# WeaponizedSchizophrenia/physically-based-renderer

Hardware: AMD Instinct MI355X
Metric: Mpaths/s + HBM GB/s (% of peak), 1920x1080x1024 spp glTF scene (higher is better)
Workload: dtype f32

## Files before the change

physically-based-renderer_amd/csrc/pt_kernels.hip:

```cpp
#include "pt_device.h"
#include "ptc_internal.h"

#ifndef TRACE_BLOCK
#define TRACE_BLOCK 256
#endif
#ifndef TRACE_MIN_WAVES
#define TRACE_MIN_WAVES 8
#endif
#define TRACE_WAVES (TRACE_BLOCK / 64)
#ifndef TRACE_CHUNK
#define TRACE_CHUNK 512u
#endif
#ifndef TRACE_CHUNK_SHORT
#define TRACE_CHUNK_SHORT 64u
#endif
#ifndef TRACE_REFILL_IDLE
#define TRACE_REFILL_IDLE 1
#endif
#ifndef TRACE_RING
#define TRACE_RING 64
#endif
#define RING_FIELDS 5
#ifndef TRACE_NODE_MIN
#define TRACE_NODE_MIN 40
#endif
#ifndef TRACE_NODE_MIN_ANY
#define TRACE_NODE_MIN_ANY TRACE_NODE_MIN
#endif
#ifndef SHADE_BLOCK
#define SHADE_BLOCK 256
#endif
#ifndef SHADE_MIN_WAVES
#define SHADE_MIN_WAVES 4
#endif
#define SHADE_WAVES (SHADE_BLOCK / 64)
#define SHADE_LDS_LIGHTS 64
#define SHADE_LDS_MATS 64
#define SHADE_LDS_ENV_ROWS 2048
#define HIT_CLASS_SHIFT 28

PT_DEV uint32_t wave_fetch(uint32_t* ctr, uint32_t amount, uint32_t lane) {
  uint32_t base = 0;
  if (lane == 0) base = atomicAdd(ctr, amount);
  return (uint32_t)__builtin_amdgcn_readfirstlane((int)base);
}
PT_DEV unsigned long long wave_sum(unsigned long long v) {
  for (int o = 32; o > 0; o >>= 1) v += __shfl_xor(v, o);
  return v;
}

#define SCAN_BLOCK 1024
PT_DEV uint32_t block_sum_1024(uint32_t v, uint32_t* s_w , uint32_t& excl) {
  const uint32_t lane = lane_id(), wave = threadIdx.x >> 6;
  uint32_t inc = v;
#pragma unroll
  for (int o = 1; o < 64; o <<= 1) { const uint32_t t = __shfl_up(inc, o); if ((int)lane >= o) inc += t; }
  __syncthreads();
  if (lane == 63) s_w[wave] = inc;
  __syncthreads();
  uint32_t before = 0, total = 0;
#pragma unroll
  for (uint32_t w = 0; w < SCAN_BLOCK / 64; ++w) { const uint32_t t = s_w[w]; if (w < wave) before += t; total += t; }
  excl = before + inc - v;
  return total;
}
PT_DEV void scan_chunks(const uint32_t* seg, uint32_t n_seg, uint32_t* pre, uint32_t* hdr, uint32_t trace_waves, uint32_t* s_w) {
  const uint32_t per = (n_seg + SCAN_BLOCK - 1u) / SCAN_BLOCK;
  const uint32_t s0 = threadIdx.x * per, s1 = s0 + per < n_seg ? s0 + per : n_seg;
  uint32_t mine = 0, dummy;
  for (uint32_t sg = s0; sg < s1; ++sg) mine += seg[sg];
  const uint32_t total = block_sum_1024(mine, s_w, dummy);
  const uint32_t per_wave = (total + trace_waves - 1u) / trace_waves;
  const uint32_t chunk = per_wave >= TRACE_CHUNK ? TRACE_CHUNK : TRACE_CHUNK_SHORT;
  uint32_t chunks = 0;
  for (uint32_t sg = s0; sg < s1; ++sg) chunks += (seg[sg] + chunk - 1u) / chunk;
  uint32_t run;
  const uint32_t all = block_sum_1024(chunks, s_w, run);
  for (uint32_t sg = s0; sg < s1; ++sg) { pre[sg] = run; run += (seg[sg] + chunk - 1u) / chunk; }
  if (threadIdx.x == 0) { pre[n_seg] = all; hdr[0] = total; hdr[1] = chunk; hdr[2] = all; }
}
__global__ __launch_bounds__(SCAN_BLOCK) void k_set_counts(DevQueues q, uint32_t n_rays, uint32_t n_shadow, uint32_t trace_waves) {
  __shared__ uint32_t s_w[SCAN_BLOCK / 64];
  for (uint32_t sg = threadIdx.x; sg < q.n_seg; sg += SCAN_BLOCK) {
    const uint64_t lo = (uint64_t)sg * q.seg_len;
    q.seg_ray[0][sg] = lo >= n_rays ? 0u : (n_rays - lo > q.seg_len ? q.seg_len : (uint32_t)(n_rays - lo));
    q.seg_ray[1][sg] = 0u;
    q.seg_sh[sg] = lo >= n_shadow ? 0u : (n_shadow - lo > q.seg_len ? q.seg_len : (uint32_t)(n_shadow - lo));
  }
  __syncthreads();
  scan_chunks(q.seg_ray[0], q.n_seg, q.pre_ray, &q.cnt[CNT_RAY_TOTAL], trace_waves, s_w);
  scan_chunks(q.seg_sh, q.n_seg, q.pre_sh, &q.cnt[CNT_SH_TOTAL], trace_waves, s_w);
  if (threadIdx.x == 0) { q.cnt[CNT_WORK_TRACE] = 0; q.cnt[CNT_WORK_SHADOW] = 0; }
}
__global__ __launch_bounds__(SCAN_BLOCK) void k_scan(DevQueues q, int qi_next, uint32_t trace_waves) {
  __shared__ uint32_t s_w[SCAN_BLOCK / 64];
  scan_chunks(q.seg_ray[qi_next], q.n_seg, q.pre_ray, &q.cnt[CNT_RAY_TOTAL], trace_waves, s_w);
  scan_chunks(q.seg_sh, q.n_seg, q.pre_sh, &q.cnt[CNT_SH_TOTAL], trace_waves, s_w);
  if (threadIdx.x == 0) { q.cnt[CNT_WORK_TRACE] = 0; q.cnt[CNT_WORK_SHADOW] = 0; }
}

template <bool RASTER>
__global__ __launch_bounds__(256) void k_raygen(DevCamera cam, DevFrame fr, DevQueues q, uint32_t first_sample, uint32_t n_paths) {
  const uint32_t p = blockIdx.x * 256u + threadIdx.x;
  if (p >= n_paths) return;
  const uint32_t j = p % fr.n_owned, sl = p / fr.n_owned;
  const uint32_t pixel = fr.owned[j];
  const uint32_t px = pixel % (uint32_t)fr.w, py = pixel / (uint32_t)fr.w;
  const uint32_t sample = first_sample + sl;
  const uint32_t key = path_key(fr.seed_hash, pixel, sample);
  float jx = 0.5f, jy = 0.5f;
  if (!RASTER) { jx = rng_f(key, 0, 0); jy = rng_f(key, 0, 1); }
  const float fx = ((float)px + jx) / (float)fr.w, fy = ((float)py + jy) / (float)fr.h;
  const float dvx = (2.0f * fx - 1.0f) * cam.sx, dvy = (2.0f * fy - 1.0f) * cam.sy;
  const v3 cs = V3(cam.s[0], cam.s[1], cam.s[2]), cu = V3(cam.u[0], cam.u[1], cam.u[2]), cf = V3(cam.f[0], cam.f[1], cam.f[2]);
  const v3 d = normalize3(vfma(cs, dvx, vfma(cu, dvy, cf)));
  float bz = 1.0f, bw = 1.0f;
  if (RASTER) {
    const float len = pt_sqrt(pt_fma(dvy, dvy, pt_fma(dvx, dvx, 1.0f)));
    const float dnear = (2.0f * PT_ZFAR * PT_ZNEAR) / (PT_ZFAR + PT_ZNEAR);
    bz = dnear * len; bw = PT_ZFAR * len;
  }
  const RayQ& r = q.ray[0];
  r.A[p] = make_float4(cam.pos[0], cam.pos[1], cam.pos[2], d.x);
  r.B[p] = make_float4(d.y, d.z, bz, bw);
  r.C[p] = make_float4(1.0f, 0.0f, __uint_as_float(p), __uint_as_float(key));
  q.lpath[p] = make_float4(0.0f, 0.0f, 0.0f, 0.0f);
}

struct WStack {
  typedef unsigned int ux2 __attribute__((ext_vector_type(2)));
  typedef __attribute__((address_space(3))) ux2 lds_u2;
  typedef __attribute__((address_space(1))) ux2 glb_u2;
  lds_u2* lds; glb_u2* ovf; int sp; int L;
  PT_DEV void init(uint2* lds_base, uint2* ovf_wave, int l) { lds = (lds_u2*)lds_base; ovf = (glb_u2*)ovf_wave; sp = 0; L = l; }
  PT_DEV void reset() { sp = 0; }
  PT_DEV void push(uint32_t base, uint32_t mask) {
    const ux2 e = {base, mask};
    if (sp < L) lds[sp * 64] = e; else ovf[(sp - L) * 64 + (int)lane_id()] = e;
    ++sp;
  }
  PT_DEV uint2 pop() {
    --sp;
    ux2 e;
    if (sp < L) e = lds[sp * 64]; else e = ovf[(sp - L) * 64 + (int)lane_id()];
    return make_uint2(e.x, e.y);
  }
  PT_DEV bool empty() const { return sp == 0; }
};

typedef float float2v __attribute__((ext_vector_type(2)));
PT_DEV float hw_max(float a, float b) { return __builtin_fmaxf(a, b); }
PT_DEV float hw_min(float a, float b) { return __builtin_fminf(a, b); }
PT_DEV float ubyte_f(uint32_t w, int i) { return (float)((w >> (8 * i)) & 255u); }

#define CUR_DONE ((int)0x80000000)
#define CUR_FINISHED (CUR_DONE + 1)
#define CUR_LEAF (CUR_DONE + 2)

PT_DEV uint32_t ray_octant(const ray_t& r) { return (r.inv.x >= 0.0f ? 1u : 0u) | (r.inv.y >= 0.0f ? 2u : 0u) | (r.inv.z >= 0.0f ? 4u : 0u); }

#define ORDER_TABLE_BYTES 2048
PT_DEV void build_order_table(uint8_t* tab) {
  for (uint32_t i = threadIdx.x; i < ORDER_TABLE_BYTES; i += TRACE_BLOCK) {
    const uint32_t oct = i >> 8, hits = i & 255u;
    uint32_t best = 0, bk = 0;
    for (uint32_t sl = 0; sl < 8u; ++sl)
      if ((hits >> sl) & 1u) { const uint32_t k = (sl ^ oct) + 1u; if (k > bk) { bk = k; best = sl; } }
    tab[i] = (uint8_t)best;
  }
}

PT_DEV uint32_t node_visit(const DevScene& sc, uint32_t node_addr, int cur, const ray_t& r, uint32_t oct, float tmin, float tlimit,
                           uint32_t& block, uint32_t& masks) {
  typedef float fx4 __attribute__((ext_vector_type(4)));
  typedef __attribute__((address_space(3))) const fx4 lds_f4;
  typedef __attribute__((address_space(1))) const fx4 glb_f4;
  fx4 f0, f1, f2, f3;
  if ((uint32_t)cur < sc.n_lds_units) {
    lds_f4* p = (lds_f4*)(uintptr_t)node_addr;
    f0 = p[0]; f1 = p[1]; f2 = p[2]; f3 = p[3];
  } else {
    glb_f4* p = (glb_f4*)sc.recs + (uint32_t)cur;
    f0 = p[0]; f1 = p[1]; f2 = p[2]; f3 = p[3];
  }
  const uint32_t w0 = __float_as_uint(f0.x), w1 = __float_as_uint(f0.y), w2 = __float_as_uint(f0.z);
  const float ox = pt_fma((float)(w0 & 0xffffu), sc.grid_step[0], sc.grid_lo[0]), oy = pt_fma((float)(w0 >> 16), sc.grid_step[1], sc.grid_lo[1]),
              oz = pt_fma((float)(w1 & 0xffffu), sc.grid_step[2], sc.grid_lo[2]);
  const float ax = __uint_as_float(((w1 >> 16) & 255u) << 23) * r.inv.x, ay = __uint_as_float((w1 >> 24) << 23) * r.inv.y,
              az = __uint_as_float((w2 & 255u) << 23) * r.inv.z;
  const float bx = pt_fma(ox, r.inv.x, -(r.o.x * r.inv.x)), by = pt_fma(oy, r.inv.y, -(r.o.y * r.inv.y)), bz = pt_fma(oz, r.inv.z, -(r.o.z * r.inv.z));
  const bool px = (oct & 1u) != 0u, py = (oct & 2u) != 0u, pz = (oct & 4u) != 0u;
  const uint32_t lx[2] = {__float_as_uint(f1.x), __float_as_uint(f1.y)}, ly[2] = {__float_as_uint(f1.z), __float_as_uint(f1.w)},
                 lz[2] = {__float_as_uint(f2.x), __float_as_uint(f2.y)}, hx[2] = {__float_as_uint(f2.z), __float_as_uint(f2.w)},
                 hy[2] = {__float_as_uint(f3.x), __float_as_uint(f3.y)}, hz[2] = {__float_as_uint(f3.z), __float_as_uint(f3.w)};
  uint32_t hits = 0;
#pragma unroll
  for (int h = 1; h >= 0; --h) {
    const uint32_t nqx = px ? lx[h] : hx[h], fqx = px ? hx[h] : lx[h];
    const uint32_t nqy = py ? ly[h] : hy[h], fqy = py ? hy[h] : ly[h];
    const uint32_t nqz = pz ? lz[h] : hz[h], fqz = pz ? hz[h] : lz[h];
#pragma unroll
    for (int i = 3; i >= 0; --i) {
      const float tn = hw_max(hw_max(hw_max(pt_fma(ubyte_f(nqx, i), ax, bx), pt_fma(ubyte_f(nqy, i), ay, by)), pt_fma(ubyte_f(nqz, i), az, bz)), tmin);
      const float tf = hw_min(hw_min(hw_min(pt_fma(ubyte_f(fqx, i), ax, bx), pt_fma(ubyte_f(fqy, i), ay, by)), pt_fma(ubyte_f(fqz, i), az, bz)), tlimit);
#ifndef PT_NO_ADDC
// ... 33 lines not shown
  const uint32_t second = tmask >> 24;
  const uint32_t k = tbase + 3u * ((uint32_t)__builtin_popcount((tmask >> 8) & 255u & below) + (uint32_t)__builtin_popcount((tmask >> 16) & 255u & below) + second);
  const bool more = second == 0u && ((tmask >> (16u + sl)) & 1u) != 0u;
  tmask = more ? (tmask | (1u << 24)) : ((tmask & 0x00ffffffu) & ~(1u << sl));
  return k;
}

PT_DEV uint32_t pending_triangles(uint32_t tmask) {
  const uint32_t lh = tmask & 255u;
  return (uint32_t)__builtin_popcount(lh) + (uint32_t)__builtin_popcount((tmask >> 16) & lh) - (tmask >> 24);
}
#ifndef LEAF_EXTRA
#define LEAF_EXTRA 1
#endif
struct LeafDeal { uint32_t off, take, ntask, rank_free; bool helper; };
PT_DEV LeafDeal leaf_deal(uint32_t extra, bool leaf, uint64_t m_leaf) {
  LeafDeal d;
  uint32_t off = 0, total = 0;
#pragma unroll
  for (int b = 0; (1 << b) <= LEAF_EXTRA; ++b) {
    const uint64_t m = __ballot(((extra >> b) & 1u) != 0u);
    off += mbcnt64(m) << b; total += (uint32_t)__popcll(m) << b;
  }
  const uint64_t m_free = ~m_leaf;
  const uint32_t n_free = (uint32_t)__popcll(m_free);
  d.rank_free = mbcnt64(m_free);
  d.ntask = total < n_free ? total : n_free;
  d.helper = !leaf && d.rank_free < d.ntask;
  d.off = off;
  d.take = off >= d.ntask ? 0u : (d.ntask - off < extra ? d.ntask - off : extra);
  return d;
}

struct Reservoir {
  uint32_t next, end, n_chunks, chunk, my_static; bool exhausted, static_left;
  PT_DEV void init(const uint32_t* hdr, uint32_t wave_in_grid) {
    chunk = hdr[1]; n_chunks = hdr[2];
    my_static = wave_in_grid; static_left = wave_in_grid < n_chunks;
    next = end = 0; exhausted = false;
  }
  static PT_DEV bool block_has_no_work(const uint32_t* hdr) { return hdr[2] <= blockIdx.x * TRACE_WAVES; }
  PT_DEV void open_chunk(const DevQueues& q, const uint32_t* pre, const uint32_t* seg, uint32_t c, uint32_t lane) {
    uint32_t lo = 0, span = q.n_seg;
    while (span > 1u) {
      const uint32_t step = (span + 63u) >> 6, idx = lo + lane * step;
      const uint32_t v = lane * step < span ? pre[idx] : 0xffffffffu;
      const uint32_t k = (uint32_t)__popcll(__ballot(v <= c)) - 1u;
      lo += k * step;
      span = span - k * step < step ? span - k * step : step;
    }
    const uint32_t first = pre[lo], cnt = seg[lo];
    const uint32_t j = c - (uint32_t)__builtin_amdgcn_readfirstlane((int)first), live = (uint32_t)__builtin_amdgcn_readfirstlane((int)cnt);
    lo = (uint32_t)__builtin_amdgcn_readfirstlane((int)lo);
    next = lo * q.seg_len + j * chunk;
    end = lo * q.seg_len + ((j + 1u) * chunk < live ? (j + 1u) * chunk : live);
  }
  PT_DEV uint32_t take(const DevQueues& q, const uint32_t* pre, const uint32_t* seg, uint32_t* ctr, uint32_t lane, uint32_t want, uint32_t& first) {
    if (next >= end && !exhausted) {
      if (chunk < TRACE_CHUNK) {
        if (my_static < n_chunks) { open_chunk(q, pre, seg, my_static, lane); my_static += gridDim.x * TRACE_WAVES; }
        else exhausted = true;
      } else if (static_left) { static_left = false; open_chunk(q, pre, seg, my_static, lane); }
      else {
        const uint32_t waves = gridDim.x * TRACE_WAVES;
        if (n_chunks <= waves) exhausted = true;
        else {
          const uint64_t c = (uint64_t)waves + wave_fetch(ctr, 1u, lane);
          if (c >= n_chunks) exhausted = true; else open_chunk(q, pre, seg, (uint32_t)c, lane);
        }
      }
    }
    const uint32_t avail = end - next;
    const uint32_t n = avail < want ? avail : want;
    first = next; next += n;
    return n;
  }
};

struct RayRing {
  typedef __attribute__((address_space(3))) uint32_t lds_u32;
  lds_u32* f;
  uint32_t n;
  PT_DEV void init(uint32_t* base) { f = (lds_u32*)base; n = 0; }
  PT_DEV void stage(Reservoir& res, const DevQueues& q, const uint32_t* pre, const uint32_t* seg, uint32_t* ctr, const float4* QA, const float4* QB, uint32_t lane) {
    uint32_t first;
    const uint32_t k = res.take(q, pre, seg, ctr, lane, TRACE_RING, first);
    if (lane < k) {
      const uint32_t ri = first + lane;
      const float4 A = QA[ri], B = QB[ri];
      const ray_t r = make_ray(V3(A.x, A.y, A.z), V3(A.w, B.x, B.y));
      f[lane] = ri;
      f[TRACE_RING + lane] = __float_as_uint(r.inv.x); f[2 * TRACE_RING + lane] = __float_as_uint(r.inv.y); f[3 * TRACE_RING + lane] = __float_as_uint(r.inv.z);
      f[4 * TRACE_RING + lane] = (r.inv.x >= 0.0f ? 1u : 0u) | (r.inv.y >= 0.0f ? 2u : 0u) | (r.inv.z >= 0.0f ? 4u : 0u);
    }
    n = (uint32_t)__builtin_amdgcn_readfirstlane((int)k);
    __builtin_amdgcn_fence(__ATOMIC_RELEASE, "wavefront");
    __builtin_amdgcn_wave_barrier();
    __builtin_amdgcn_fence(__ATOMIC_ACQUIRE, "wavefront");
  }
  PT_DEV bool pop(bool idle, uint32_t& ri, v3& inv, uint32_t& oct) {
    const uint64_t m = __ballot(idle);
    const uint32_t rank = mbcnt64(m), need = (uint32_t)__popcll(m);
    const bool got = idle && rank < n;
    if (got) {
      const uint32_t i = n - 1u - rank;
      ri = f[i];
      inv = V3(__uint_as_float(f[TRACE_RING + i]), __uint_as_float(f[2 * TRACE_RING + i]), __uint_as_float(f[3 * TRACE_RING + i]));
      oct = f[4 * TRACE_RING + i];
    }
    n -= need < n ? need : n;
    return got;
  }
};

#ifdef PT_DIAG
#define DIAG_ITER(var) do { const uint64_t m_ = __ballot(true); if ((int)lane == __ffsll((unsigned long long)m_) - 1) ++(var); } while (0)
#else
#define DIAG_ITER(var) do { } while (0)
#endif

struct TraceLds { uint32_t top_addr; uint2* stack; uint8_t* order_tab; uint32_t* ring; };
PT_DEV TraceLds trace_lds(float4* lds_raw, const DevScene& sc, int stack_lds, bool closest) {
  TraceLds t;
  t.top_addr = (uint32_t)(uintptr_t)(__attribute__((address_space(3))) void*)lds_raw;
  t.stack = reinterpret_cast<uint2*>(lds_raw + sc.n_lds_units);
  t.order_tab = reinterpret_cast<uint8_t*>(t.stack + (size_t)TRACE_WAVES * (size_t)stack_lds * 64u);
  t.ring = reinterpret_cast<uint32_t*>(t.order_tab + (closest ? ORDER_TABLE_BYTES : 0));
  return t;
}
PT_DEV void load_triangle(const DevScene& sc, uint32_t top_addr, uint32_t k, float4& a, float4& b, float4& c) {
  typedef float fx4 __attribute__((ext_vector_type(4)));
  typedef __attribute__((address_space(3))) const fx4 lds_f4;
  typedef __attribute__((address_space(1))) const fx4 glb_f4;
  fx4 x, y, z;
  if (k + 3u <= sc.n_lds_units) { lds_f4* p = (lds_f4*)(uintptr_t)(top_addr + 16u * k); x = p[0]; y = p[1]; z = p[2]; }
  else { glb_f4* p = (glb_f4*)sc.recs + k; x = p[0]; y = p[1]; z = p[2]; }
  a = make_float4(x.x, x.y, x.z, x.w); b = make_float4(y.x, y.y, y.z, y.w); c = make_float4(z.x, z.y, z.z, z.w);
}

template <bool CULL>
__global__ __launch_bounds__(TRACE_BLOCK, TRACE_MIN_WAVES) void k_trace_closest(DevScene sc, DevQueues q, int qi, int stack_lds) {
  extern __shared__ float4 lds_raw[];
  __shared__ uint8_t s_pair[2][TRACE_WAVES][64];
  const uint32_t lane = lane_id();
  const uint32_t wave = threadIdx.x >> 6;
  if (Reservoir::block_has_no_work(&q.cnt[CNT_RAY_TOTAL])) return;
  const TraceLds L = trace_lds(lds_raw, sc, stack_lds, true);
  uint8_t* order_tab = L.order_tab;
  for (uint32_t i = threadIdx.x; i < sc.n_lds_units; i += TRACE_BLOCK) lds_raw[i] = sc.recs[i];
  build_order_table(order_tab);
  __syncthreads();
  const RayQ rq = q.ray[qi];
  unsigned long long nv = 0, nr = 0, nh = 0;
  uint32_t nt = 0;
  uint32_t d_node = 0, d_tri = 0, d_round = 0, d_leftpass = 0, d_left = 0;
  (void)d_node; (void)d_tri; (void)d_round; (void)d_leftpass; (void)d_left;
#ifdef PT_STAMP
  unsigned long long t_refill = 0, t_node = 0, t_leaf = 0, t_fin = 0, t_mark = __builtin_amdgcn_s_memtime();
#define STAMP(acc) do { __builtin_amdgcn_sched_barrier(0); const unsigned long long t_ = __builtin_amdgcn_s_memtime(); acc += t_ - t_mark; t_mark = t_; __builtin_amdgcn_sched_barrier(0); } while (0)
#else
#define STAMP(acc) do { } while (0)
#endif
  Reservoir res; res.init(&q.cnt[CNT_RAY_TOTAL], (uint32_t)__builtin_amdgcn_readfirstlane((int)(blockIdx.x * TRACE_WAVES + wave)));
  const uint32_t* seg_cnt = q.seg_ray[qi];
  WStack st;
  st.init(L.stack + (size_t)wave * (size_t)stack_lds * 64u + lane,
          sc.stack_ovf + ((size_t)__builtin_amdgcn_readfirstlane((int)(blockIdx.x * TRACE_WAVES + wave)) * sc.ovf_depth) * 64u, stack_lds);
  int cur = CUR_DONE;
  uint32_t ri = 0, oct = 0, gbase = 0, gmask = 0, tbase = 0, tmask = 0;
  ray_t r = make_ray(V3(0, 0, 0), V3(0, 0, 1));
  float tmin = 0.0f, best_t = PT_T_INF, best_u = 0.0f, best_v = 0.0f;
  int best_prim = 0x7fffffff, best_cls = 0;
  bool found = false;
  RayRing ring; ring.init(L.ring + (size_t)wave * RING_FIELDS * TRACE_RING);
  for (;;) {
    {
      bool idle = cur == CUR_DONE;
      uint64_t mi = __ballot(idle);
      if ((uint32_t)__popcll(mi) >= TRACE_REFILL_IDLE || !__ballot(cur != CUR_DONE)) {
        while (mi) {
          if (ring.n == 0u) {
            if (res.exhausted) break;
            ring.stage(res, q, q.pre_ray, seg_cnt, &q.cnt[CNT_WORK_TRACE], rq.A, rq.B, lane);
            if (ring.n == 0u) break;
          }
          v3 inv = V3(0, 0, 0); uint32_t oc = 0;
          const bool got = ring.pop(idle, ri, inv, oc);
          nr += (unsigned long long)__popcll(__ballot(got));
          if (got) {
            const float4 A = rq.A[ri], Bq = rq.B[ri];
            r.o = V3(A.x, A.y, A.z); r.d = V3(A.w, Bq.x, Bq.y); r.inv = inv;
            oct = oc;
            tmin = CULL ? Bq.z : 0.0f;
            best_t = CULL ? Bq.w : PT_T_INF; best_u = 0.0f; best_v = 0.0f; best_prim = 0x7fffffff; best_cls = 0; found = false;
            st.reset();
            gmask = 0; tmask = 0;
            cur = 0;
          }
          idle = cur == CUR_DONE; mi = __ballot(idle);
        }
      }
    }
    STAMP(t_refill);
    if (!__ballot(cur != CUR_DONE)) break;
    DIAG_ITER(d_round);
    {
      for (;;) {
        const uint64_t mn = __ballot(cur >= 0);
        if (!mn) break;
        if (__popcll(mn) < TRACE_NODE_MIN && __ballot(cur == CUR_LEAF)) break;
        nv += (unsigned long long)__popcll(mn);
        if (cur >= 0) {
          DIAG_ITER(d_node);
          uint32_t nb, masks;
          const uint32_t node_addr = L.top_addr + 16u * (uint32_t)cur;
          const uint32_t hits = node_visit(sc, node_addr, cur, r, oct, tmin, best_t, nb, masks);
          const uint32_t imask = masks & 255u, lhits = hits & (masks >> 8);
          enter_group(gbase, gmask, st, nb, hits & imask, imask);
          tbase = nb + 4u * (uint32_t)__builtin_popcount(imask);
          tmask = lhits | (masks & 0x00ffff00u);
          cur = lhits ? CUR_LEAF : advance<true>(gbase, gmask, st, order_tab, oct);
        }
      }
      STAMP(t_node);
#if LEAF_EXTRA == 0
      {
        const bool leaf = cur == CUR_LEAF;
        if (__ballot(leaf)) {
          DIAG_ITER(d_tri);
          if (leaf) {
            const uint32_t k = next_triangle(tbase, tmask);
            float4 a, b, c;
            load_triangle(sc, L.top_addr, k, a, b, c);
            float t, u, v;
            const bool hit = tri_test<CULL>(r, V3(a.x, a.y, a.z), V3(b.x, b.y, b.z), V3(c.x, c.y, c.z), t, u, v);
            const int pid = __float_as_int(a.w);
            ++nt;
            if (hit && t > tmin && (t < best_t || (t == best_t && pid < best_prim))) {
              best_t = t; best_u = u; best_v = v; best_prim = pid; best_cls = __float_as_int(b.w); found = true;
            }
            if ((tmask & 255u) == 0u) cur = advance<true>(gbase, gmask, st, order_tab, oct);
          }
        }
      }
#elif LEAF_EXTRA > 1
      {
        const bool leaf = cur == CUR_LEAF;
        const uint64_t m_leaf = __ballot(leaf);
        if (m_leaf) {
          DIAG_ITER(d_tri);
          uint32_t k1 = 0, pend = 0;
          if (leaf) { k1 = next_triangle(tbase, tmask); pend = pending_triangles(tmask); }
          const LeafDeal dl = leaf_deal(pend < LEAF_EXTRA ? pend : LEAF_EXTRA, leaf, m_leaf);
          typedef __attribute__((address_space(3))) volatile uint8_t lds_u8;
          lds_u8* tab_task = (lds_u8*)s_pair[0][wave];
          lds_u8* tab_helper = (lds_u8*)s_pair[1][wave];
          uint32_t kx[LEAF_EXTRA];
#pragma unroll
          for (uint32_t j = 0; j < LEAF_EXTRA; ++j) {
            kx[j] = 0;
            if (j < dl.take) { kx[j] = next_triangle(tbase, tmask); tab_task[dl.off + j] = (uint8_t)(lane | (j << 6)); }
          }
          if (dl.helper) tab_helper[dl.rank_free] = (uint8_t)lane;
          __builtin_amdgcn_fence(__ATOMIC_RELEASE, "wavefront");
          __builtin_amdgcn_wave_barrier();
          __builtin_amdgcn_fence(__ATOMIC_ACQUIRE, "wavefront");
          const uint32_t task = dl.helper ? (uint32_t)tab_task[dl.rank_free] : lane;
          const int src = (int)(task & 63u);
          ray_t rr;
          rr.o = V3(__shfl(r.o.x, src), __shfl(r.o.y, src), __shfl(r.o.z, src));
          rr.d = V3(__shfl(r.d.x, src), __shfl(r.d.y, src), __shfl(r.d.z, src));
          uint32_t k = k1;
#pragma unroll
          for (uint32_t j = 0; j < LEAF_EXTRA; ++j) {
            const uint32_t kj = (uint32_t)__shfl((int)kx[j], src);
            if (dl.helper && (task >> 6) == j) k = kj;
          }
          bool hit = false; float t = 0.0f, u = 0.0f, v = 0.0f; int pid = 0, cls = 0;
          if (leaf || dl.helper) {
            float4 a, b, c;
            load_triangle(sc, L.top_addr, k, a, b, c);
            hit = tri_test<CULL>(rr, V3(a.x, a.y, a.z), V3(b.x, b.y, b.z), V3(c.x, c.y, c.z), t, u, v);
            pid = __float_as_int(a.w); cls = __float_as_int(b.w);
          }
          if (leaf) {
            ++nt;
            if (hit && t > tmin && (t < best_t || (t == best_t && pid < best_prim))) {
              best_t = t; best_u = u; best_v = v; best_prim = pid; best_cls = cls; found = true;
            }
          }
          const float tt = hit ? t : -INFINITY;
          const int pw = pid | (cls << HIT_CLASS_SHIFT);
          float bt = 0.0f; int bp = 0, bl = (int)lane; bool have = false;
#pragma unroll
          for (uint32_t j = 0; j < LEAF_EXTRA; ++j) {
            const int hl = j < dl.take ? (int)tab_helper[dl.off + j] : (int)lane;
            const float tj = __shfl(tt, hl);
            const int pj = __shfl(pw, hl);
            if (j < dl.take) {
              ++nt;
              const int prim_j = pj & ((1 << HIT_CLASS_SHIFT) - 1);
              if (tj > tmin && (!have || tj < bt || (tj == bt && prim_j < (bp & ((1 << HIT_CLASS_SHIFT) - 1))))) { bt = tj; bp = pj; bl = hl; have = true; }
            }
          }
          const float ub = __shfl(u, bl), vb = __shfl(v, bl);
          if (have) {
            const int prim_b = bp & ((1 << HIT_CLASS_SHIFT) - 1);
            if (bt < best_t || (bt == best_t && prim_b < best_prim)) {
              best_t = bt; best_u = ub; best_v = vb; best_prim = prim_b; best_cls = (int)((uint32_t)bp >> HIT_CLASS_SHIFT); found = true;
            }
          }
          if (leaf && (tmask & 255u) == 0u) cur = advance<true>(gbase, gmask, st, order_tab, oct);
#ifdef PT_DIAG
          {
            const uint32_t left = (cur == CUR_LEAF) ? pending_triangles(tmask) : 0u;
            const uint64_t m_left = __ballot(left != 0u);
            if (m_left) { if ((int)lane == __ffsll((unsigned long long)m_left) - 1) ++d_leftpass; d_left += left; }
          }
#endif
        }
      }
#else
      {
        const bool leaf = cur == CUR_LEAF;
        const uint64_t m_leaf = __ballot(leaf);
        if (m_leaf) {
          DIAG_ITER(d_tri);
          uint32_t k1 = 0, k2 = 0;
          bool more = false;
          if (leaf) { k1 = next_triangle(tbase, tmask); more = (tmask & 255u) != 0u; }
          const uint64_t m_more = __ballot(more), m_free = ~m_leaf;
          const uint32_t n_more = (uint32_t)__popcll(m_more), n_free = (uint32_t)__popcll(m_free);
          const uint32_t rank_more = mbcnt64(m_more), rank_free = mbcnt64(m_free);
          const bool paired = more && rank_more < n_free, helper = !leaf && rank_free < n_more;
          typedef __attribute__((address_space(3))) volatile uint8_t lds_u8;
          lds_u8* tab_owner = (lds_u8*)s_pair[0][wave];
          lds_u8* tab_helper = (lds_u8*)s_pair[1][wave];
          if (paired) { k2 = next_triangle(tbase, tmask); tab_owner[rank_more] = (uint8_t)lane; }
          if (helper) tab_helper[rank_free] = (uint8_t)lane;
          __builtin_amdgcn_fence(__ATOMIC_RELEASE, "wavefront");
          __builtin_amdgcn_wave_barrier();
          __builtin_amdgcn_fence(__ATOMIC_ACQUIRE, "wavefront");
          const int src = helper ? (int)tab_owner[rank_free] : (int)lane;
          ray_t rr;
          rr.o = V3(__shfl(r.o.x, src), __shfl(r.o.y, src), __shfl(r.o.z, src));
          rr.d = V3(__shfl(r.d.x, src), __shfl(r.d.y, src), __shfl(r.d.z, src));
          const uint32_t k2_src = (uint32_t)__shfl((int)k2, src);
          const uint32_t k = helper ? k2_src : k1;
          bool hit = false; float t = 0.0f, u = 0.0f, v = 0.0f; int pid = 0, cls = 0;
          if (leaf || helper) {
            float4 a, b, c;
            load_triangle(sc, L.top_addr, k, a, b, c);
            hit = tri_test<CULL>(rr, V3(a.x, a.y, a.z), V3(b.x, b.y, b.z), V3(c.x, c.y, c.z), t, u, v);
            pid = __float_as_int(a.w); cls = __float_as_int(b.w);
          }
          if (leaf) {
            ++nt;
            if (hit && t > tmin && (t < best_t || (t == best_t && pid < best_prim))) {
              best_t = t; best_u = u; best_v = v; best_prim = pid; best_cls = cls; found = true;
            }
          }
          const int hsrc = paired ? (int)tab_helper[rank_more] : (int)lane;
          const int h2 = __shfl(hit ? 1 : 0, hsrc);
          const float t2 = __shfl(t, hsrc), u2 = __shfl(u, hsrc), v2 = __shfl(v, hsrc);
          const int pid2 = __shfl(pid, hsrc), cls2 = __shfl(cls, hsrc);
          if (paired) {
            ++nt;
            if (h2 && t2 > tmin && (t2 < best_t || (t2 == best_t && pid2 < best_prim))) {
              best_t = t2; best_u = u2; best_v = v2; best_prim = pid2; best_cls = cls2; found = true;
            }
          }
          if (leaf && (tmask & 255u) == 0u) cur = advance<true>(gbase, gmask, st, order_tab, oct);
#ifdef PT_DIAG
          {
            const uint32_t left = (cur == CUR_LEAF) ? (uint32_t)__builtin_popcount(tmask & 255u) + (uint32_t)__builtin_popcount((tmask >> 16) & tmask & 255u) - (tmask >> 24) : 0u;
            const uint64_t m_left = __ballot(left != 0u);
            if (m_left) { if ((int)lane == __ffsll((unsigned long long)m_left) - 1) ++d_leftpass; d_left += left; }
          }
#endif
        }
      }
#endif
      STAMP(t_leaf);
      nh += (unsigned long long)__popcll(__ballot(cur == CUR_FINISHED && found));
      if (cur == CUR_FINISHED) {
        q.hit[ri] = make_float4(found ? best_t : -1.0f, __int_as_float(found ? (best_prim | (best_cls << HIT_CLASS_SHIFT)) : -1), best_u, best_v);
        cur = CUR_DONE;
      }
      STAMP(t_fin);
    }
  }
  {
    __shared__ unsigned long long s_stat[TRACE_WAVES][4];
    const unsigned long long c_tris = wave_sum(nt);
    if (lane == 0) { s_stat[wave][0] = nv; s_stat[wave][1] = c_tris; s_stat[wave][2] = nr; s_stat[wave][3] = nh; }
    __syncthreads();
    if (threadIdx.x < 4u) {
      unsigned long long v = 0;
      for (int w = 0; w < TRACE_WAVES; ++w) v += s_stat[w][threadIdx.x];
      const int at = threadIdx.x == 0u ? ST_NODES_C : threadIdx.x == 1u ? ST_TRIS_C : threadIdx.x == 2u ? ST_SEGMENTS : ST_HITS;
      if (v) atomicAdd(&q.stats[at * ST_STRIDE], v);
    }
  }
#ifdef PT_STAMP
  if (lane == 0) { atomicAdd(&q.stats[ST_DIAG_NODE_ITERS * ST_STRIDE], t_node); atomicAdd(&q.stats[ST_DIAG_TRI_ITERS * ST_STRIDE], t_leaf); atomicAdd(&q.stats[ST_DIAG_LEAF_VISITS * ST_STRIDE], t_fin); atomicAdd(&q.stats[ST_DIAG_ROUNDS * ST_STRIDE], t_refill); }
#endif
#ifdef PT_DIAG
  {
    unsigned long long a0 = wave_sum(d_node), a1 = wave_sum(d_tri), a3 = wave_sum(d_round), a4 = wave_sum(d_leftpass), a5 = wave_sum(d_left);
    if (lane == 0) { atomicAdd(&q.stats[ST_DIAG_NODE_ITERS * ST_STRIDE], a0); atomicAdd(&q.stats[ST_DIAG_TRI_ITERS * ST_STRIDE], a1); atomicAdd(&q.stats[ST_DIAG_ROUNDS * ST_STRIDE], a3);
                     atomicAdd(&q.stats[ST_DIAG_LEAF_VISITS * ST_STRIDE], a4); atomicAdd(&q.stats[ST_DIAG_REFILLED * ST_STRIDE], a5); }
  }
#endif
}

template <bool DEBUG_OUT>
__global__ __launch_bounds__(TRACE_BLOCK, TRACE_MIN_WAVES) void k_trace_any(DevScene sc, DevQueues q, int stack_lds, uint8_t* debug_out) {
  extern __shared__ float4 lds_raw[];
  __shared__ uint8_t s_pair[2][TRACE_WAVES][64];
  const uint32_t lane = lane_id();
  const uint32_t wave = threadIdx.x >> 6;
  if (Reservoir::block_has_no_work(&q.cnt[CNT_SH_TOTAL])) return;
  const TraceLds L = trace_lds(lds_raw, sc, stack_lds, false);
  for (uint32_t i = threadIdx.x; i < sc.n_lds_units; i += TRACE_BLOCK) lds_raw[i] = sc.recs[i];
  __syncthreads();
  unsigned long long nv = 0, nr = 0;
  uint32_t nt = 0;
  Reservoir res; res.init(&q.cnt[CNT_SH_TOTAL], (uint32_t)__builtin_amdgcn_readfirstlane((int)(blockIdx.x * TRACE_WAVES + wave)));
  WStack st;
  st.init(L.stack + (size_t)wave * (size_t)stack_lds * 64u + lane,
          sc.stack_ovf + ((size_t)__builtin_amdgcn_readfirstlane((int)(blockIdx.x * TRACE_WAVES + wave)) * sc.ovf_depth) * 64u, stack_lds);
  int cur = CUR_DONE;
  uint32_t ri = 0, path = 0, oct = 0, gbase = 0, gmask = 0, tbase = 0, tmask = 0;
  ray_t r = make_ray(V3(0, 0, 0), V3(0, 0, 1));
  float tmax = 0.0f;
  bool occluded = false;
  RayRing ring; ring.init(L.ring + (size_t)wave * RING_FIELDS * TRACE_RING);
  for (;;) {
    {
      bool idle = cur == CUR_DONE;
      uint64_t mi = __ballot(idle);
      if ((uint32_t)__popcll(mi) >= TRACE_REFILL_IDLE || !__ballot(cur != CUR_DONE)) {
        while (mi) {
          if (ring.n == 0u) {
            if (res.exhausted) break;
            ring.stage(res, q, q.pre_sh, q.seg_sh, &q.cnt[CNT_WORK_SHADOW], q.shadow.A, q.shadow.B, lane);
            if (ring.n == 0u) break;
          }
          v3 inv = V3(0, 0, 0); uint32_t oc = 0;
          const bool got = ring.pop(idle, ri, inv, oc);
          nr += (unsigned long long)__popcll(__ballot(got));
          if (got) {
            const float4 A = q.shadow.A[ri], Bq = q.shadow.B[ri];
            r.o = V3(A.x, A.y, A.z); r.d = V3(A.w, Bq.x, Bq.y); r.inv = inv;
            oct = oc;
            tmax = Bq.z; path = __float_as_uint(Bq.w);
            occluded = false;
            st.reset();
            gmask = 0; tmask = 0;
            cur = 0;
          }
          idle = cur == CUR_DONE; mi = __ballot(idle);
        }
      }
    }
    if (!__ballot(cur != CUR_DONE)) break;
    {
      for (;;) {
        const uint64_t mn = __ballot(cur >= 0);
        if (!mn) break;
        if (__popcll(mn) < TRACE_NODE_MIN_ANY && __ballot(cur == CUR_LEAF)) break;
        nv += (unsigned long long)__popcll(mn);
        if (cur >= 0) {
          uint32_t nb, masks;
          const uint32_t node_addr = L.top_addr + 16u * (uint32_t)cur;
          const uint32_t hits = node_visit(sc, node_addr, cur, r, oct, 0.0f, tmax, nb, masks);
          const uint32_t imask = masks & 255u, lhits = hits & (masks >> 8);
          enter_group(gbase, gmask, st, nb, hits & imask, imask);
          tbase = nb + 4u * (uint32_t)__builtin_popcount(imask);
          tmask = lhits | (masks & 0x00ffff00u);
          cur = lhits ? CUR_LEAF : advance<false>(gbase, gmask, st, nullptr, 0u);
        }
      }
#if LEAF_EXTRA == 0
      {
        const bool leaf = cur == CUR_LEAF;
        if (__ballot(leaf)) {
          if (leaf) {
            const uint32_t k = next_triangle(tbase, tmask);
            float4 a, b, c;
            load_triangle(sc, L.top_addr, k, a, b, c);
            float t, u, v;
            const bool hit = tri_test<false>(r, V3(a.x, a.y, a.z), V3(b.x, b.y, b.z), V3(c.x, c.y, c.z), t, u, v) && t > 0.0f && t < tmax;
            ++nt;
            if (hit) { occluded = true; cur = CUR_FINISHED; }
            else if ((tmask & 255u) == 0u) cur = advance<false>(gbase, gmask, st, nullptr, 0u);
          }
        }
      }
#elif LEAF_EXTRA > 1
      {
        const bool leaf = cur == CUR_LEAF;
        const uint64_t m_leaf = __ballot(leaf);
        if (m_leaf) {
          uint32_t k1 = 0, pend = 0;
          if (leaf) { k1 = next_triangle(tbase, tmask); pend = pending_triangles(tmask); }
          const LeafDeal dl = leaf_deal(pend < LEAF_EXTRA ? pend : LEAF_EXTRA, leaf, m_leaf);
          typedef __attribute__((address_space(3))) volatile uint8_t lds_u8;
          lds_u8* tab_task = (lds_u8*)s_pair[0][wave];
          lds_u8* tab_helper = (lds_u8*)s_pair[1][wave];
          uint32_t kx[LEAF_EXTRA];
#pragma unroll
          for (uint32_t j = 0; j < LEAF_EXTRA; ++j) {
            kx[j] = 0;
            if (j < dl.take) { kx[j] = next_triangle(tbase, tmask); tab_task[dl.off + j] = (uint8_t)(lane | (j << 6)); }
          }
          if (dl.helper) tab_helper[dl.rank_free] = (uint8_t)lane;
          __builtin_amdgcn_fence(__ATOMIC_RELEASE, "wavefront");
          __builtin_amdgcn_wave_barrier();
          __builtin_amdgcn_fence(__ATOMIC_ACQUIRE, "wavefront");
          const uint32_t task = dl.helper ? (uint32_t)tab_task[dl.rank_free] : lane;
          const int src = (int)(task & 63u);
          ray_t rr;
          rr.o = V3(__shfl(r.o.x, src), __shfl(r.o.y, src), __shfl(r.o.z, src));
          rr.d = V3(__shfl(r.d.x, src), __shfl(r.d.y, src), __shfl(r.d.z, src));
          const float tmax_src = __shfl(tmax, src);
          uint32_t k = k1;
#pragma unroll
          for (uint32_t j = 0; j < LEAF_EXTRA; ++j) {
// ... 183 lines not shown
  if (y0 < 0) y0 += si.z;
  if (x1 > si.y - 1) x1 -= si.y;
  if (y1 > si.z - 1) y1 -= si.z;
  const uint4 t00 = ldu4(sc.set_texels, set_texel_at(si, x0, y0)), t10 = ldu4(sc.set_texels, set_texel_at(si, x1, y0)),
              t01 = ldu4(sc.set_texels, set_texel_at(si, x0, y1)), t11 = ldu4(sc.set_texels, set_texel_at(si, x1, y1));
  auto bil = [&](uint32_t p00, uint32_t p10, uint32_t p01, uint32_t p11) {
    const float4 c00 = unorm8x4(p00), c10 = unorm8x4(p10), c01 = unorm8x4(p01), c11 = unorm8x4(p11);
    const float ax = pt_fma(tx, c10.x - c00.x, c00.x), ay = pt_fma(tx, c10.y - c00.y, c00.y), az = pt_fma(tx, c10.z - c00.z, c00.z), aw = pt_fma(tx, c10.w - c00.w, c00.w);
    const float bx = pt_fma(tx, c11.x - c01.x, c01.x), by = pt_fma(tx, c11.y - c01.y, c01.y), bz = pt_fma(tx, c11.z - c01.z, c01.z), bw = pt_fma(tx, c11.w - c01.w, c01.w);
    return make_float4(pt_fma(ty, bx - ax, ax), pt_fma(ty, by - ay, ay), pt_fma(ty, bz - az, az), pt_fma(ty, bw - aw, aw));
  };
  c = bil(t00.x, t10.x, t01.x, t11.x); n = bil(t00.y, t10.y, t01.y, t11.y); m = bil(t00.z, t10.z, t01.z, t11.z);
}

template <class S> PT_DEV void apply_textures(const S& sc, float4 t0, float4 t1, float4 t2, float4 t3, float4 t4, float4 t5, float hu, float hv, float hw, float4 M2, int set, v3 ni, float base[4],
                           float& metallic, float& roughness, v3& ns) {
  const int tex_color = __float_as_int(M2.y), tex_normal = __float_as_int(M2.z), tex_mr = __float_as_int(M2.w);
  const float tu = pt_fma(t1.x, hv, pt_fma(t0.z, hu, t0.x * hw)), tv = pt_fma(t1.y, hv, pt_fma(t0.w, hu, t0.y * hw));
  float4 cc = make_float4(1, 1, 1, 1), cn = make_float4(0.5f, 0.5f, 1.0f, 1.0f), cm = make_float4(1, 1, 1, 1);
  const int4 si = ldi4(sc.set_info, (size_t)(set < 0 ? 0 : set));
  if (set >= 0 && si.x >= 0) set_fetch(sc, si, tu, tv, cc, cn, cm);
  else {
    if (tex_color >= 0) cc = tex_fetch(sc, tex_color, tu, tv);
    if (tex_mr >= 0) cm = tex_fetch(sc, tex_mr, tu, tv);
    if (tex_normal >= 0) cn = tex_fetch(sc, tex_normal, tu, tv);
  }
  if (tex_color >= 0) { base[0] = base[0] * cc.x; base[1] = base[1] * cc.y; base[2] = base[2] * cc.z; base[3] = base[3] * cc.w; }
  if (tex_mr >= 0) { roughness = roughness * cm.y; metallic = metallic * cm.z; }
  if (tex_normal >= 0) {
    const float nx = 2.0f * cn.x - 1.0f, ny = 2.0f * cn.y - 1.0f, nz = 2.0f * cn.z - 1.0f;
    const v3 ti = V3(pt_fma(t3.x, hv, pt_fma(t2.y, hu, t1.z * hw)), pt_fma(t3.y, hv, pt_fma(t2.z, hu, t1.w * hw)), pt_fma(t3.z, hv, pt_fma(t2.w, hu, t2.x * hw)));
    const v3 bi = V3(pt_fma(t5.y, hv, pt_fma(t4.z, hu, t3.w * hw)), pt_fma(t5.z, hv, pt_fma(t4.w, hu, t4.x * hw)), pt_fma(t5.w, hv, pt_fma(t5.x, hu, t4.y * hw)));
    ns = normalize3(vfma(ti, nx, vfma(bi, ny, ni * nz)));
  }
}

template <class S> PT_DEV void env_lookup(const S& sc, v3 d, v3& Le, float& pdf) {
  const float u = pt_atan2(d.z, d.x) * (0.5f * PT_INV_PI) + 0.5f;
  const float dy = fmin2(fmax2(d.y, -1.0f), 1.0f);
  const float st = pt_sqrt(fmax2(0.0f, 1.0f - dy * dy));
  const float vv = pt_atan2(st, dy) * PT_INV_PI;
  int x = (int)(u * (float)sc.env_w), y = (int)(vv * (float)sc.env_h);
  if (x > sc.env_w - 1) x = sc.env_w - 1;
  if (x < 0) x = 0;
  if (y > sc.env_h - 1) y = sc.env_h - 1;
  if (y < 0) y = 0;
  const float4 t = ld4(sc.env, (size_t)y * (size_t)sc.env_w + (size_t)x);
  Le = V3(t.x, t.y, t.z);
  pdf = sc.env_ok ? (t.w * (float)sc.env_w * (float)sc.env_h) / (2.0f * PT_PI * PT_PI * fmax2(st, 1e-6f)) : 0.0f;
}
template <class P> PT_DEV uint32_t cdf_search(const P& cdf, uint32_t n, float r) {
  uint32_t lo = 0, hi = n - 1u;
  while (lo < hi) { const uint32_t mid = (lo + hi) >> 1; if (cdf[mid] > r) hi = mid; else lo = mid + 1u; }
  return lo;
}
template <class P, class G> PT_DEV uint32_t cdf_search_guided(const P& cdf, const G& guide, float r) {
  const uint32_t b = (uint32_t)(r * (float)PTC_ENV_GUIDE);
  uint32_t lo = guide[b], hi = guide[b + 1u];
  while (lo < hi) { const uint32_t mid = (lo + hi) >> 1; if (cdf[mid] > r) hi = mid; else lo = mid + 1u; }
  return lo;
}
template <class S, class P, class G> PT_DEV v3 env_sample(const S& sc, const P& marg, const G& marg_guide, float r1, float r2) {
  const uint32_t y = cdf_search_guided(marg, marg_guide, r1);
  const float m0 = y ? marg[y - 1u] : 0.0f, m1 = marg[y];
  float xi_v = m1 > m0 ? (r1 - m0) / (m1 - m0) : 0.5f;
  const auto cc = sc.env_cond + (size_t)y * (size_t)sc.env_w;
  const uint32_t x = cdf_search_guided(cc, sc.env_cond_guide + (size_t)y * (PTC_ENV_GUIDE + 1u), r2);
  const float c0 = x ? cc[x - 1u] : 0.0f, c1 = cc[x];
  float xi_u = c1 > c0 ? (r2 - c0) / (c1 - c0) : 0.5f;
  xi_u = fmin2(fmax2(xi_u, 0.0f), 0.999999f); xi_v = fmin2(fmax2(xi_v, 0.0f), 0.999999f);
  const float u = ((float)x + xi_u) / (float)sc.env_w, vv = ((float)y + xi_v) / (float)sc.env_h;
  float s2, c2, st, ct;
  sincos2pi(u, s2, c2);
  sincos2pi(0.5f * vv, st, ct);
  return V3(st * -c2, ct, st * -s2);
}

#define SHADE_RING 128
PT_DEV void wave_lds_sync() {
  __builtin_amdgcn_fence(__ATOMIC_RELEASE, "wavefront");
  __builtin_amdgcn_wave_barrier();
  __builtin_amdgcn_fence(__ATOMIC_ACQUIRE, "wavefront");
}
template <bool SORT, bool TABLES_LDS>
__global__ __launch_bounds__(SHADE_BLOCK, SHADE_MIN_WAVES) void k_shade(const DevScene* __restrict__ scp, DevFrame fr, DevQueues q, int qi, uint32_t b) {
  __shared__ float4 s_light[SHADE_LDS_LIGHTS * 5];
  __shared__ float s_cdf[SHADE_LDS_LIGHTS];
  __shared__ float4 s_mat[SHADE_LDS_MATS * 4];
  __shared__ uint32_t s_ring[SORT ? SHADE_WAVES : 1][PTC_MATERIAL_CLASSES][SORT ? SHADE_RING : 1];
  __shared__ float s_marg[SHADE_LDS_ENV_ROWS];
  __shared__ uint16_t s_marg_guide[PTC_ENV_GUIDE + 2];
  const DevScene& dsc = *scp;
  const GScene sc = global_view(dsc);
  const uint32_t lane = lane_id();
  const uint32_t wave = threadIdx.x >> 6;
  const bool lds_lights = TABLES_LDS || sc.n_lights <= SHADE_LDS_LIGHTS, lds_mats = TABLES_LDS || sc.n_mats <= SHADE_LDS_MATS;
  if (lds_lights) {
    for (uint32_t i = threadIdx.x; i < sc.n_lights * 5u; i += SHADE_BLOCK) s_light[i] = ld4((AS_GLOBAL const fx4*)dsc.lights, i);
    for (uint32_t i = threadIdx.x; i < sc.n_lights; i += SHADE_BLOCK) s_cdf[i] = ((AS_GLOBAL const float*)dsc.cdf)[i];
  }
  if (lds_mats)
    for (uint32_t i = threadIdx.x; i < sc.n_mats * 4u; i += SHADE_BLOCK) s_mat[i] = ld4((AS_GLOBAL const fx4*)dsc.mats, i);
  const bool lds_marg = sc.env_ok != 0 && (TABLES_LDS || sc.env_h <= SHADE_LDS_ENV_ROWS);
  if (lds_marg) {
    for (uint32_t i = threadIdx.x; i < (uint32_t)sc.env_h; i += SHADE_BLOCK) s_marg[i] = ((AS_GLOBAL const float*)dsc.env_marg)[i];
    for (uint32_t i = threadIdx.x; i <= PTC_ENV_GUIDE; i += SHADE_BLOCK) s_marg_guide[i] = ((AS_GLOBAL const uint16_t*)dsc.env_marg_guide)[i];
  }
  __syncthreads();
  const Dual<float, TABLES_LDS> env_marg = {(AS_LDS const float*)s_marg, (AS_GLOBAL const float*)dsc.env_marg, lds_marg};
  const Dual<uint16_t, TABLES_LDS> env_marg_guide = {(AS_LDS const uint16_t*)s_marg_guide, (AS_GLOBAL const uint16_t*)dsc.env_marg_guide, lds_marg};
  const uint32_t seg = blockIdx.x * SHADE_WAVES + wave;
  if (seg >= q.n_seg) return;
  const Dual<fx4, TABLES_LDS> lights = {(AS_LDS const fx4*)s_light, (AS_GLOBAL const fx4*)dsc.lights, lds_lights};
  const Dual<float, TABLES_LDS> cdf = {(AS_LDS const float*)s_cdf, (AS_GLOBAL const float*)dsc.cdf, lds_lights};
  const Dual<fx4, TABLES_LDS> mats = {(AS_LDS const fx4*)s_mat, (AS_GLOBAL const fx4*)dsc.mats, lds_mats};
  const bool has_env = sc.env_w > 0, env_nee = has_env && sc.env_ok != 0;
  const float p_env = env_nee ? (sc.n_lights > 0u ? 0.5f : 1.0f) : 0.0f, p_area = 1.0f - p_env;
  const RayQ rin = q.ray[qi], rout = q.ray[qi ^ 1];
  const uint32_t base = seg * q.seg_len;
  const uint32_t n = (uint32_t)__builtin_amdgcn_readfirstlane((int)q.seg_ray[qi][seg]);
  typedef __attribute__((address_space(3))) volatile uint32_t lds_u32;
  lds_u32* ring = (lds_u32*)&s_ring[SORT ? wave : 0][0][0];
#ifdef PT_STAMP_SHADE
  unsigned long long t_front = 0, t_load = 0, t_math = 0, t_back = 0, t_mark = __builtin_amdgcn_s_memtime();
#define SSTAMP(acc) do { __builtin_amdgcn_sched_barrier(0); const unsigned long long t_ = __builtin_amdgcn_s_memtime(); acc += t_ - t_mark; t_mark = t_; __builtin_amdgcn_sched_barrier(0); } while (0)
#define SSTAMP_LOADS(acc) do { asm volatile("s_waitcnt vmcnt(0)" ::: "memory"); SSTAMP(acc); } while (0)
#else
#define SSTAMP(acc) do { } while (0)
#define SSTAMP_LOADS(acc) do { } while (0)
#endif
  uint32_t out_a = 0, out_s = 0;
  uint32_t fillv = 0;
  uint32_t ready = 0, nonempty = 0;
  uint32_t i0 = 0;
  int w_pref = SORT && lane < n ? __float_as_int(q.hit[base + lane].y) : -1;
  for (;;) {
    bool valid; uint32_t item = 0u;
    if (!SORT) {
      if (i0 >= n) break;
      valid = i0 + lane < n; item = i0 + lane;
      i0 += 64u;
    } else {
    if (!ready) {
      if (i0 < n) {
        const uint32_t i = i0 + lane;
        int cls = -1;
        if (i < n) cls = w_pref >= 0 ? ((w_pref >> HIT_CLASS_SHIFT) & (PTC_MATERIAL_CLASSES - 1)) : (has_env ? PTC_MATERIAL_CLASSES - 1 : -1);
#ifdef SHADE_TWO_RING
        if (cls >= 0) cls = (cls >= 2 && cls != PTC_MATERIAL_CLASSES - 1) ? 1 : 0;
#endif
        i0 += 64u;
        w_pref = i0 + lane < n ? __float_as_int(q.hit[base + i0 + lane].y) : -1;
        uint64_t rem = __ballot(cls >= 0);
        while (rem) {
          const int c = __builtin_amdgcn_readlane(cls, __ffsll((unsigned long long)rem) - 1);
          const uint64_t m = __ballot(cls == c);
          uint32_t f = (uint32_t)__builtin_amdgcn_readlane((int)fillv, c);
          if (cls == c) ring[(uint32_t)c * SHADE_RING + f + mbcnt64(m)] = i;
          f += (uint32_t)__popcll(m);
          if (lane == (uint32_t)c) fillv = f;
          nonempty |= 1u << c;
          if (f >= 64u) ready |= 1u << c;
          rem &= ~m;
        }
        SSTAMP(t_front);
        continue;
      }
      if (!nonempty) break;
    }
    wave_lds_sync();
    if (ready) {
      const uint32_t c = (uint32_t)__builtin_ctz(ready);
      const uint32_t f = (uint32_t)__builtin_amdgcn_readlane((int)fillv, (int)c);
      const uint32_t rest = f - 64u;
      valid = true;
      item = ring[c * SHADE_RING + rest + lane];
      if (lane == c) fillv = rest;
      ready &= ~(1u << c);
      if (!rest) nonempty &= ~(1u << c);
    } else {
      uint32_t off = 0, left = nonempty;
      valid = false;
      while (left && off < 64u) {
        const uint32_t c = (uint32_t)__builtin_ctz(left);
        const uint32_t f = (uint32_t)__builtin_amdgcn_readlane((int)fillv, (int)c);
        const uint32_t take = f < 64u - off ? f : 64u - off;
        if (lane >= off && lane < off + take) { item = ring[c * SHADE_RING + f - take + (lane - off)]; valid = true; }
        if (lane == c) fillv = f - take;
        if (f == take) nonempty &= ~(1u << c);
        left &= ~(1u << c);
        off += take;
      }
    }
    }
    const uint32_t slot = base + item;
    SSTAMP(t_front);

    bool alive = false, has_shadow = false;
    float4 oA, oB, oC, sA, sB, sC;
    oA = oB = oC = sA = sB = sC = make_float4(0, 0, 0, 0);
    if (valid) {
      const float4 A = rin.A[slot], Bq = rin.B[slot], Cq = rin.C[slot], H = q.hit[slot];
      const v3 d = V3(A.w, Bq.x, Bq.y);
      v3 T = V3(Bq.z, Bq.w, Cq.x);
      const float prev_pdf = Cq.y;
      const uint32_t path = __float_as_uint(Cq.z), key = __float_as_uint(Cq.w);
      const float ht = H.x, hu = H.z, hv = H.w;
      if (__float_as_int(H.y) < 0) {
        if (SORT || has_env) {
        v3 Le; float pe; env_lookup(sc, d, Le, pe);
        float wgt = 1.0f;
        if (b > 0u) { const float pl = pe * p_env; const float pb2 = prev_pdf * prev_pdf; wgt = pb2 / pt_fma(pl, pl, pb2); }
        float4 L = q.lpath[path];
        L.x = pt_fma(T.x * Le.x, wgt, L.x); L.y = pt_fma(T.y * Le.y, wgt, L.y); L.z = pt_fma(T.z * Le.z, wgt, L.z);
        q.lpath[path] = L;
        }
      } else {
      const uint32_t prim = (uint32_t)__float_as_int(H.y) & ((1u << HIT_CLASS_SHIFT) - 1u);
      const size_t rec = (size_t)prim * sc.shade_stride;
      const float4 r0 = ld4(sc.shade, rec), r1 = ld4(sc.shade, rec + 1), r2 = ld4(sc.shade, rec + 2), r3 = ld4(sc.shade, rec + 3), r4 = ld4(sc.shade, rec + 4);
      const bool tex_cls = ((uint32_t)__float_as_int(H.y) >> HIT_CLASS_SHIFT) >= 2u;
      float4 x0, x1, x2, x3, x4, x5;
      x0 = x1 = x2 = x3 = x4 = x5 = make_float4(0, 0, 0, 0);
      if (tex_cls) { x0 = ld4(sc.shade, rec + 5); x1 = ld4(sc.shade, rec + 6); x2 = ld4(sc.shade, rec + 7); x3 = ld4(sc.shade, rec + 8); x4 = ld4(sc.shade, rec + 9); x5 = ld4(sc.shade, rec + 10); }
      const uint32_t rb = b + 1u;
      bool use_env = false;
      if ((int)b < fr.max_bounces && env_nee) use_env = sc.n_lights == 0u || rng_f(key, rb, 7) < p_env;
      v3 wi_env = V3(0, 0, 0);
#ifdef SHADE_ENV_ALWAYS
      if ((int)b < fr.max_bounces && env_nee) wi_env = env_sample(sc, env_marg, env_marg_guide, rng_f(key, rb, 1), rng_f(key, rb, 2));
#else
      if (use_env) wi_env = env_sample(sc, env_marg, env_marg_guide, rng_f(key, rb, 1), rng_f(key, rb, 2));
#endif
      SSTAMP_LOADS(t_load);
      const v3 Pa = V3(r0.x, r0.y, r0.z), Pb = V3(r1.x, r1.y, r1.z), Pc = V3(r2.x, r2.y, r2.z);
      const v3 Na = V3(r2.w, r3.x, r3.y), Nb = V3(r3.z, r3.w, r4.x), Nc = V3(r4.y, r4.z, r4.w);
      const float hw = 1.0f - hu - hv;
      const v3 P = V3(pt_fma(Pc.x, hv, pt_fma(Pb.x, hu, Pa.x * hw)), pt_fma(Pc.y, hv, pt_fma(Pb.y, hu, Pa.y * hw)), pt_fma(Pc.z, hv, pt_fma(Pb.z, hu, Pa.z * hw)));
      v3 ng = normalize3(cross3(Pb - Pa, Pc - Pa));
      const v3 ni = V3(pt_fma(Nc.x, hv, pt_fma(Nb.x, hu, Na.x * hw)), pt_fma(Nc.y, hv, pt_fma(Nb.y, hu, Na.y * hw)), pt_fma(Nc.z, hv, pt_fma(Nb.z, hu, Na.z * hw)));
      v3 ns = normalize3(ni);
      const int mat = __float_as_int(r0.w);
      const float4 M0 = ld4(mats, (size_t)(mat * 4 + 0)), M1 = ld4(mats, (size_t)(mat * 4 + 1)), M2 = ld4(mats, (size_t)(mat * 4 + 2));
      float base_c[4] = {M0.x, M0.y, M0.z, M2.x};
      float metallic = M0.w, roughness = M1.w;
      const bool lambert = metallic == 0.0f && roughness >= 1.0f && __float_as_int(M2.w) < 0;
      if (__float_as_int(M2.y) >= 0 || __float_as_int(M2.z) >= 0 || __float_as_int(M2.w) >= 0)
        apply_textures(sc, x0, x1, x2, x3, x4, x5, hu, hv, hw, M2, __float_as_int(ld4(mats, (size_t)(mat * 4 + 3)).x), ni, base_c, metallic, roughness, ns);
      const v3 wo = -d;
      const bool front = dot3(ng, wo) > 0.0f;
      if (dot3(ns, ng) < 0.0f) ns = -ns;
      if (!front) { ng = -ng; ns = -ns; }
      if (!(dot3(ns, wo) > 0.0f)) ns = ng;
      const int li = __float_as_int(r1.w);
      if (li >= 0 && front) {
        const float4 l0 = ld4(lights, (size_t)(li * 5 + 0)), l1 = ld4(lights, (size_t)(li * 5 + 1)), l4 = ld4(lights, (size_t)(li * 5 + 4));
        float wgt = 1.0f;
        if (b > 0u) {
          const float cosl = dot3(ng, wo);
          const float pl = ((l1.w * (ht * ht)) / (l0.w * cosl)) * p_area;
          const float pb2 = prev_pdf * prev_pdf;
          wgt = pb2 / pt_fma(pl, pl, pb2);
        }
        float4 L = q.lpath[path];
        L.x = pt_fma(T.x * l4.x, wgt, L.x); L.y = pt_fma(T.y * l4.y, wgt, L.y); L.z = pt_fma(T.z * l4.z, wgt, L.z);
        q.lpath[path] = L;
      }
      if ((int)b < fr.max_bounces) {
        const bsdf_t bs = make_bsdf(V3(base_c[0], base_c[1], base_c[2]), metallic, roughness, lambert);
        v3 tx, ty; onb(ns, tx, ty);
        const v3 wol = V3(dot3(tx, wo), dot3(ty, wo), dot3(ns, wo));
        const float ps = spec_prob(bs, fmax2(wol.z, 1e-4f));
        const v3 porg = vfma(ng, sc.ray_eps, P);
        if (use_env) {
          const v3 wi = wi_env;
          const v3 wil = V3(dot3(tx, wi), dot3(ty, wi), dot3(ns, wi));
          if (wil.z > 0.0f && dot3(ng, wi) > 0.0f) {
            v3 Le; float pe; env_lookup(sc, wi, Le, pe);
            const float pl = pe * p_env;
            if (pl > 0.0f) {
              v3 f; float pb; bsdf_eval(bs, wol, wil, ps, f, pb);
              const float pl2 = pl * pl;
              const float wgt = pl2 / pt_fma(pb, pb, pl2);
              const float k = (wil.z * wgt) / pl;
              has_shadow = true;
              sA = make_float4(porg.x, porg.y, porg.z, wi.x);
              sB = make_float4(wi.y, wi.z, PT_T_INF, __uint_as_float(path));
              sC = make_float4(T.x * f.x * Le.x * k, T.y * f.y * Le.y * k, T.z * f.z * Le.z * k, 0.0f);
            }
          }
        } else if (sc.n_lights > 0u) {
          const float u0 = rng_f(key, rb, 0), r1 = rng_f(key, rb, 1), r2 = rng_f(key, rb, 2);
          const uint32_t lo = cdf_search(cdf, sc.n_lights, u0);
          const float4 l0 = ld4(lights, (size_t)(lo * 5 + 0)), l1 = ld4(lights, (size_t)(lo * 5 + 1)), l2 = ld4(lights, (size_t)(lo * 5 + 2)), l3 = ld4(lights, (size_t)(lo * 5 + 3)), l4 = ld4(lights, (size_t)(lo * 5 + 4));
          const float su = pt_sqrt(r1);
          const float bu = su * (1.0f - r2), bv = su * r2;
          const v3 y = vfma(V3(l2.x, l2.y, l2.z), bv, vfma(V3(l1.x, l1.y, l1.z), bu, V3(l0.x, l0.y, l0.z)));
          const v3 dv = y - P;
          const float dist2 = dot3(dv, dv);
          if (dist2 > 0.0f) {
            const float dist = pt_sqrt(dist2);
            const v3 wi = dv * (1.0f / dist);
            const float cosl = -dot3(V3(l3.x, l3.y, l3.z), wi);
            const v3 wil = V3(dot3(tx, wi), dot3(ty, wi), dot3(ns, wi));
            if (cosl > 0.0f && wil.z > 0.0f && dot3(ng, wi) > 0.0f) {
              const float pl = ((l1.w * dist2) / (l0.w * cosl)) * p_area;
              v3 f; float pb; bsdf_eval(bs, wol, wil, ps, f, pb);
              const float pl2 = pl * pl;
              const float wgt = pl2 / pt_fma(pb, pb, pl2);
              const float k = (wil.z * wgt) / pl;
              has_shadow = true;
              const v3 sv = y - porg;
              const float sd = pt_sqrt(dot3(sv, sv));
              const v3 sdir = sv * (1.0f / sd);
              sA = make_float4(porg.x, porg.y, porg.z, sdir.x);
              sB = make_float4(sdir.y, sdir.z, sd * 0.999f, __uint_as_float(path));
              sC = make_float4(T.x * f.x * l4.x * k, T.y * f.y * l4.y * k, T.z * f.z * l4.z * k, 0.0f);
            }
          }
        }
        const float ul = rng_f(key, rb, 3), s1 = rng_f(key, rb, 4), s2 = rng_f(key, rb, 5);
        v3 wil;
        bool ok = bsdf_sample(bs, wol, ps, ul, s1, s2, wil);
        v3 wi = V3(0, 0, 0); float pdf = 0.0f;
        if (ok) {
          wi = vfma(tx, wil.x, vfma(ty, wil.y, ns * wil.z));
          ok = dot3(ng, wi) > 0.0f;
        }
        if (ok) {
          v3 f; bsdf_eval(bs, wol, wil, ps, f, pdf);
          ok = pdf > 0.0f;
          if (ok) {
            const float k = wil.z / pdf;
            T = V3(T.x * f.x * k, T.y * f.y * k, T.z * f.z * k);
          }
        }
        if (ok && rb >= PT_RR_START) {
          const float qq = max3c(T);
          ok = qq > 0.0f;
          if (ok) {
            const float pr = fmin2(fmax2(qq, PT_RR_PMIN), 1.0f);
            const float ur = rng_f(key, rb, 6);
            ok = !(ur >= pr);
            if (ok) T = V3(T.x / pr, T.y / pr, T.z / pr);
          }
        }
        if (ok) {
          alive = true;
          oA = make_float4(porg.x, porg.y, porg.z, wi.x);
          oB = make_float4(wi.y, wi.z, T.x, T.y);
// ... 51 lines not shown
  const int pc = __float_as_int(H.y);
  if (pc >= 0) {
    const int prim = pc & ((1 << HIT_CLASS_SHIFT) - 1);
    const float hu = H.z, hv = H.w, hw = 1.0f - hu - hv;
    const float4* rec = sc.shade + (size_t)prim * sc.shade_stride;
    const float4 r0 = rec[0], r1 = rec[1], r2 = rec[2], r3 = rec[3], r4 = rec[4];
    v3 P = V3(pt_fma(r2.x, hv, pt_fma(r1.x, hu, r0.x * hw)), pt_fma(r2.y, hv, pt_fma(r1.y, hu, r0.y * hw)), pt_fma(r2.z, hv, pt_fma(r1.z, hu, r0.z * hw)));
    const v3 ni = V3(pt_fma(r4.y, hv, pt_fma(r3.z, hu, r2.w * hw)), pt_fma(r4.z, hv, pt_fma(r3.w, hu, r3.x * hw)), pt_fma(r4.w, hv, pt_fma(r4.x, hu, r3.y * hw)));
    v3 N = normalize3(ni);
    const int mat = __float_as_int(r0.w);
    const float4 M0 = sc.mats[mat * 4 + 0], M1 = sc.mats[mat * 4 + 1], M2 = sc.mats[mat * 4 + 2];
    float base[4] = {M0.x, M0.y, M0.z, M2.x};
    float metallic = M0.w, roughness = M1.w;
    if (__float_as_int(M2.y) >= 0 || __float_as_int(M2.z) >= 0 || __float_as_int(M2.w) >= 0)
      apply_textures(sc, rec[5], rec[6], rec[7], rec[8], rec[9], rec[10], hu, hv, hw, M2, __float_as_int(sc.mats[mat * 4 + 3].x), ni, base, metallic, roughness, N);
    if (GBUF16) {
      P = V3(round_f16(P.x), round_f16(P.y), round_f16(P.z));
      N = V3(round_f16(N.x), round_f16(N.y), round_f16(N.z));
#pragma unroll
      for (int k = 0; k < 4; ++k) base[k] = round_unorm16(base[k]);
    }
    const v3 V = normalize3(V3(cam.pos[0], cam.pos[1], cam.pos[2]) - P);
    const v3 Hh = normalize3(V + V);
    const float ndv = fmax2(dot3(N, V), 0.0f), ndh = fmax2(dot3(N, Hh), 0.0f);
    const float s2 = ndh * ndh, s4 = s2 * s2, s8 = s4 * s4, s16 = s8 * s8, s32 = s16 * s16, spec = s32 * s32;
    o = make_float4(pt_fma(base[0], ndv, spec), pt_fma(base[1], ndv, spec), pt_fma(base[2], ndv, spec), pt_fma(base[3], ndv, spec));
  }
  accum[j] = o;
}

__global__ __launch_bounds__(256) void k_to_half(const float4* in, uint2* out, uint32_t n) {
  const uint32_t i = blockIdx.x * 256u + threadIdx.x;
  if (i >= n) return;
  const float4 c = in[i];
  const _Float16 hx = (_Float16)c.x, hy = (_Float16)c.y, hz = (_Float16)c.z, hw = (_Float16)c.w;
  const uint32_t bx = __builtin_bit_cast(unsigned short, hx), by = __builtin_bit_cast(unsigned short, hy),
                 bz = __builtin_bit_cast(unsigned short, hz), bw = __builtin_bit_cast(unsigned short, hw);
  out[i] = make_uint2(bx | (by << 16), bz | (bw << 16));
}

PT_DEV float rrt_odt(float c) {
  const float num = c * (c + 0.0245786f) - 0.000090537f;
  const float den = c * (0.983729f * c + 0.4329510f) + 0.238081f;
  return num / den;
}
__global__ __launch_bounds__(256) void k_tonemap(const float4* radiance, uint32_t* out, int w, int h) {
  const int x = blockIdx.x * 16 + (threadIdx.x & 15), y = blockIdx.y * 16 + (threadIdx.x >> 4);
  if (x >= w || y >= h) return;
  const float4 c = radiance[(size_t)y * w + x];
  const float ir = 0.59719f * c.x + 0.07600f * c.y + 0.02840f * c.z;
  const float ig = 0.35458f * c.x + 0.90834f * c.y + 0.13383f * c.z;
  const float ib = 0.04823f * c.x + 0.01566f * c.y + 0.83777f * c.z;
  const float fr = rrt_odt(ir), fg = rrt_odt(ig), fb = rrt_odt(ib);
  const float orr = 1.60475f * fr + -0.10208f * fg + -0.00327f * fb;
  const float og = -0.53108f * fr + 1.10813f * fg + -0.07276f * fb;
  const float ob = -0.07367f * fr + -0.00605f * fg + 1.07602f * fb;
  const float v4[4] = {orr, og, ob, c.w};
  uint32_t packed = 0;
#pragma unroll
  for (int k = 0; k < 4; ++k) {
    float v = v4[k];
    if (k < 3) v = pt_pow(fmax2(v, 0.0f), 1.0f / 2.2f);
    v = fmin2(fmax2(v, 0.0f), 1.0f);
    packed |= ((uint32_t)(int)(v * 255.0f + 0.5f)) << (8 * k);
  }
  out[(size_t)y * w + x] = packed;
}

static size_t trace_lds_bytes(const LaunchCfg& cfg, const DevScene& sc, bool closest) {
  return (size_t)sc.n_lds_units * 16 + (size_t)TRACE_WAVES * cfg.stack_lds * 64 * 8 + (closest ? ORDER_TABLE_BYTES : 0) + (size_t)TRACE_WAVES * RING_FIELDS * TRACE_RING * 4;
}

int pt_trace_block_threads() { return TRACE_BLOCK; }
#define PT_STR2(x) #x
#define PT_STR(x) PT_STR2(x)
const char* pt_kernel_policy() {
  return "trace_block=" PT_STR(TRACE_BLOCK) " trace_min_waves=" PT_STR(TRACE_MIN_WAVES) " chunk=" PT_STR(TRACE_CHUNK) " ring=" PT_STR(TRACE_RING) " refill_idle=" PT_STR(TRACE_REFILL_IDLE)
         " node_min=" PT_STR(TRACE_NODE_MIN) " leaf_extra=" PT_STR(LEAF_EXTRA) " shade_block=" PT_STR(SHADE_BLOCK) " shade_min_waves=" PT_STR(SHADE_MIN_WAVES);
}

size_t pt_trace_lds_bytes(const LaunchCfg& cfg, const DevScene& sc) { return trace_lds_bytes(cfg, sc, true); }

int pt_trace_blocks_per_cu(size_t lds) {
  const void* fns[] = {(const void*)k_trace_closest<false>, (const void*)k_trace_closest<true>, (const void*)k_trace_any<false>, (const void*)k_trace_any<true>};
  int best = 1 << 30;
  for (const void* f : fns) {
    if (lds > 64u * 1024u && hipFuncSetAttribute(f, hipFuncAttributeMaxDynamicSharedMemorySize, (int)lds) != hipSuccess) return -1;
    int nb = 0;
    if (hipOccupancyMaxActiveBlocksPerMultiprocessor(&nb, f, TRACE_BLOCK, lds) != hipSuccess) return -1;
    if (nb < best) best = nb;
  }
  return best;
}

static uint32_t trace_waves(const LaunchCfg& cfg) { return (uint32_t)(cfg.n_cu * cfg.trace_blocks_per_cu) * TRACE_WAVES; }
void pt_launch_set_counts(hipStream_t s, const LaunchCfg& cfg, const DevQueues& q, uint32_t n_rays, uint32_t n_shadow) {
  hipLaunchKernelGGL(k_set_counts, dim3(1), dim3(SCAN_BLOCK), 0, s, q, n_rays, n_shadow, trace_waves(cfg));
}
void pt_launch_scan(hipStream_t s, const LaunchCfg& cfg, const DevQueues& q, int qi_next) {
  hipLaunchKernelGGL(k_scan, dim3(1), dim3(SCAN_BLOCK), 0, s, q, qi_next, trace_waves(cfg));
}
int pt_shade_block_threads() { return SHADE_BLOCK; }

void pt_launch_raygen(hipStream_t s, const DevCamera& cam, const DevFrame& fr, const DevQueues& q, uint32_t first_sample, uint32_t n_samples, bool raster) {
  const uint32_t n_paths = fr.n_owned * n_samples;
  const dim3 grid((n_paths + 255u) / 256u);
  if (raster) hipLaunchKernelGGL(k_raygen<true>, grid, dim3(256), 0, s, cam, fr, q, first_sample, n_paths);
  else hipLaunchKernelGGL(k_raygen<false>, grid, dim3(256), 0, s, cam, fr, q, first_sample, n_paths);
}

void pt_launch_trace_closest(hipStream_t s, const LaunchCfg& cfg, const DevScene& sc, const DevQueues& q, int qi, bool cull) {
  const dim3 grid((unsigned)(cfg.n_cu * cfg.trace_blocks_per_cu));
  const size_t lds = trace_lds_bytes(cfg, sc, true);
  if (cull) hipLaunchKernelGGL(k_trace_closest<true>, grid, dim3(TRACE_BLOCK), lds, s, sc, q, qi, cfg.stack_lds);
  else hipLaunchKernelGGL(k_trace_closest<false>, grid, dim3(TRACE_BLOCK), lds, s, sc, q, qi, cfg.stack_lds);
}

void pt_launch_trace_any(hipStream_t s, const LaunchCfg& cfg, const DevScene& sc, const DevQueues& q, uint8_t* debug_out) {
  const dim3 grid((unsigned)(cfg.n_cu * cfg.trace_blocks_per_cu));
  const size_t lds = trace_lds_bytes(cfg, sc, false);
  if (debug_out) hipLaunchKernelGGL(k_trace_any<true>, grid, dim3(TRACE_BLOCK), lds, s, sc, q, cfg.stack_lds, debug_out);
  else hipLaunchKernelGGL(k_trace_any<false>, grid, dim3(TRACE_BLOCK), lds, s, sc, q, cfg.stack_lds, debug_out);
}

void pt_launch_shade(hipStream_t s, const LaunchCfg& cfg, const DevScene* sc, const DevFrame& fr, const DevQueues& q, int qi, uint32_t bounce) {
  const dim3 grid((q.n_seg + SHADE_WAVES - 1u) / SHADE_WAVES);
  if (cfg.shade_sort) hipLaunchKernelGGL((k_shade<true, false>), grid, dim3(SHADE_BLOCK), 0, s, sc, fr, q, qi, bounce);
  else if (cfg.shade_tables_lds) hipLaunchKernelGGL((k_shade<false, true>), grid, dim3(SHADE_BLOCK), 0, s, sc, fr, q, qi, bounce);
  else hipLaunchKernelGGL((k_shade<false, false>), grid, dim3(SHADE_BLOCK), 0, s, sc, fr, q, qi, bounce);
}
bool pt_shade_tables_fit(const DevScene& sc) {
  return sc.n_lights <= SHADE_LDS_LIGHTS && sc.n_mats <= SHADE_LDS_MATS && (!sc.env_ok || sc.env_h <= (int)SHADE_LDS_ENV_ROWS);
}
void pt_launch_accumulate(hipStream_t s, const DevFrame& fr, const DevQueues& q, float4* accum, uint32_t n_samples) {
  hipLaunchKernelGGL(k_accumulate, dim3((fr.n_owned + 255u) / 256u), dim3(256), 0, s, fr, (const float4*)q.lpath, accum, n_samples);
}
void pt_launch_shade_raster(hipStream_t s, const DevScene& sc, const DevCamera& cam, const DevFrame& fr, const DevQueues& q, float4* accum, bool gbuffer16) {
  if (gbuffer16) hipLaunchKernelGGL(k_shade_raster<true>, dim3((fr.n_owned + 255u) / 256u), dim3(256), 0, s, sc, cam, fr, q, accum);
  else hipLaunchKernelGGL(k_shade_raster<false>, dim3((fr.n_owned + 255u) / 256u), dim3(256), 0, s, sc, cam, fr, q, accum);
}
void pt_launch_to_half(hipStream_t s, const float4* radiance, uint2* out, uint32_t n_pixels) {
  hipLaunchKernelGGL(k_to_half, dim3((n_pixels + 255u) / 256u), dim3(256), 0, s, radiance, out, n_pixels);
}
void pt_launch_resolve(hipStream_t s, const DevFrame& fr, const float4* accum, float4* radiance, float spp, bool raster) {
  hipLaunchKernelGGL(k_resolve, dim3((fr.n_owned + 255u) / 256u), dim3(256), 0, s, fr, accum, radiance, spp, raster ? 1 : 0);
}
void pt_launch_tonemap(hipStream_t s, const float4* radiance, uint32_t* rgba8, int w, int h) {
  hipLaunchKernelGGL(k_tonemap, dim3((unsigned)((w + 15) / 16), (unsigned)((h + 15) / 16)), dim3(256), 0, s, radiance, rgba8, w, h);
}

PT_DEV v3 guide_dir(const DevCamera& cam, int w, int h, uint32_t pixel) {
  const uint32_t px = pixel % (uint32_t)w, py = pixel / (uint32_t)w;
  const float fx = ((float)px + 0.5f) / (float)w, fy = ((float)py + 0.5f) / (float)h;
  const float dvx = (2.0f * fx - 1.0f) * cam.sx, dvy = (2.0f * fy - 1.0f) * cam.sy;
  const v3 cs = V3(cam.s[0], cam.s[1], cam.s[2]), cu = V3(cam.u[0], cam.u[1], cam.u[2]), cf = V3(cam.f[0], cam.f[1], cam.f[2]);
  return normalize3(vfma(cs, dvx, vfma(cu, dvy, cf)));
}
__global__ __launch_bounds__(256) void k_raygen_guides(DevCamera cam, int w, int h, uint32_t first_pixel, uint32_t n, DevQueues q) {
  const uint32_t p = blockIdx.x * 256u + threadIdx.x;
  if (p >= n) return;
  const v3 d = guide_dir(cam, w, h, first_pixel + p);
  const RayQ& r = q.ray[0];
  r.A[p] = make_float4(cam.pos[0], cam.pos[1], cam.pos[2], d.x);
  r.B[p] = make_float4(d.y, d.z, 1.0f, 1.0f);
  r.C[p] = make_float4(1.0f, 0.0f, __uint_as_float(p), 0.0f);
}
__global__ __launch_bounds__(256) void k_guides(DevScene sc, DevCamera cam, int w, int h, uint32_t first_pixel, uint32_t n, const float4* hit,
                                                float4* albedo_class, float4* normal_depth, float4* pos_class, int32_t* prim_out, float2* uv_out) {
  const uint32_t j = blockIdx.x * 256u + threadIdx.x;
  if (j >= n) return;
  const uint32_t pixel = first_pixel + j;
  const float4 H = hit[j];
  const int pc = __float_as_int(H.y);
  float4 ak = make_float4(1.0f, 1.0f, 1.0f, 0.0f), nz = make_float4(0.0f, 0.0f, 0.0f, 0.0f);
  int prim = -1;
  float2 uv = make_float2(0.0f, 0.0f);
  if (pc >= 0) {
    prim = pc & ((1 << HIT_CLASS_SHIFT) - 1);
    const float hu = H.z, hv = H.w, hw = 1.0f - hu - hv;
    uv = make_float2(hu, hv);
    nz.w = H.x;
    const float4* rec = sc.shade + (size_t)prim * sc.shade_stride;
    const float4 r0 = rec[0], r2 = rec[2], r3 = rec[3], r4 = rec[4];
    const int mat = __float_as_int(r0.w);
    const float4 M0 = sc.mats[mat * 4 + 0], M1 = sc.mats[mat * 4 + 1], M2 = sc.mats[mat * 4 + 2];
    if (M1.x != 0.0f || M1.y != 0.0f || M1.z != 0.0f) ak.w = 2.0f;
    else {
      const v3 ni = V3(pt_fma(r4.y, hv, pt_fma(r3.z, hu, r2.w * hw)), pt_fma(r4.z, hv, pt_fma(r3.w, hu, r3.x * hw)), pt_fma(r4.w, hv, pt_fma(r4.x, hu, r3.y * hw)));
      const v3 N = normalize3(ni);
      v3 ns = N;
      float base[4] = {M0.x, M0.y, M0.z, M2.x};
      float metallic = M0.w, roughness = M1.w;
      if (__float_as_int(M2.y) >= 0 || __float_as_int(M2.z) >= 0 || __float_as_int(M2.w) >= 0)
        apply_textures(sc, rec[5], rec[6], rec[7], rec[8], rec[9], rec[10], hu, hv, hw, M2, __float_as_int(sc.mats[mat * 4 + 3].x), ni, base, metallic, roughness, ns);
      ak = make_float4(base[0], base[1], base[2], 1.0f);
      nz.x = N.x; nz.y = N.y; nz.z = N.z;
    }
  }
  const v3 d = guide_dir(cam, w, h, pixel);
  albedo_class[pixel] = ak;
  normal_depth[pixel] = nz;
  pos_class[pixel] = make_float4(cam.pos[0] + nz.w * d.x, cam.pos[1] + nz.w * d.y, cam.pos[2] + nz.w * d.z, ak.w);
  prim_out[pixel] = prim;
  uv_out[pixel] = uv;
}
void pt_launch_raygen_guides(hipStream_t s, const DevCamera& cam, int w, int h, uint32_t first_pixel, uint32_t n, const DevQueues& q) {
  hipLaunchKernelGGL(k_raygen_guides, dim3((n + 255u) / 256u), dim3(256), 0, s, cam, w, h, first_pixel, n, q);
}
void pt_launch_guides(hipStream_t s, const DevScene& sc, const DevCamera& cam, int w, int h, uint32_t first_pixel, uint32_t n, const DevQueues& q, const GuideBufs& g) {
  hipLaunchKernelGGL(k_guides, dim3((n + 255u) / 256u), dim3(256), 0, s, sc, cam, w, h, first_pixel, n, (const float4*)q.hit, g.albedo_class, g.normal_depth, g.pos_class, g.prim, g.uv);
}
```

physically-based-renderer_amd/csrc/ptc_api.cpp:

```cpp
#include "../../include/ptc.h"
#include "ptc_internal.h"
#include "pt_refit.h"
#include "pt_build.h"
#include "pt_denoise.h"
#include "pt_adaptive.h"
#include "pt_temporal.h"
#include "pt_deform.h"
#include "pt_lens.h"

#include <dlfcn.h>
#include <rccl/rccl.h>

#include <chrono>
#include <cmath>
#include <cstdlib>
#include <cstring>
#include <map>
#include <mutex>
#include <memory>
#include <string>
#include <vector>

#define PTC_STR2(x) #x
#define PTC_STR(x) PTC_STR2(x)
// ... 40 lines not shown
  bool tree_device_sah = false;
  std::vector<DevDeform> deform;
  std::vector<std::vector<float>> pose_stage;
  std::vector<uint32_t> mesh_first;
  HostVertex* mesh_verts_rw = nullptr;
};

struct MeshPose {
  std::shared_ptr<DeformMesh> data;
  std::shared_ptr<std::vector<HostVertex>> base;
  std::vector<float> w, J;
  std::vector<float> pose_live;
  std::shared_ptr<std::vector<HostVertex>> base_live;
  const void* base_on_device = nullptr;
  bool host_fresh = false;
  bool emis_fresh = false;
  bool dev_fresh = false;
  bool on_device = false;
  bool active() const { return base != nullptr; }
  std::vector<float> pose() const { std::vector<float> p(w); p.insert(p.end(), J.begin(), J.end()); return p; }
};

struct Rccl {
  void* so = nullptr;
  ncclResult_t (*GetUniqueId)(ncclUniqueId*) = nullptr;
  ncclResult_t (*CommInitRank)(ncclComm_t*, int, ncclUniqueId, int) = nullptr;
  ncclResult_t (*CommInitAll)(ncclComm_t*, int, const int*) = nullptr;
  ncclResult_t (*CommDestroy)(ncclComm_t) = nullptr;
  ncclResult_t (*Reduce)(const void*, void*, size_t, ncclDataType_t, ncclRedOp_t, int, ncclComm_t, hipStream_t) = nullptr;
  ncclResult_t (*GroupStart)() = nullptr;
  ncclResult_t (*GroupEnd)() = nullptr;
  const char* (*GetErrorString)(ncclResult_t) = nullptr;
  std::string err;
};
Rccl g_rccl;
bool rccl_load() {
  if (g_rccl.so) return true;
  void* so = dlopen("librccl.so.1", RTLD_NOW | RTLD_GLOBAL);
  if (!so) so = dlopen("librccl.so", RTLD_NOW | RTLD_GLOBAL);
  if (!so) so = dlopen("/opt/rocm/lib/librccl.so.1", RTLD_NOW | RTLD_GLOBAL);
  if (!so) { const char* e = dlerror(); g_rccl.err = std::string("librccl.so not loadable: ") + (e ? e : "?"); return false; }
  bool ok = true;
  auto sym = [&](const char* name) { void* p = dlsym(so, name); if (!p) { ok = false; g_rccl.err = std::string("librccl.so lacks ") + name; } return p; };
  g_rccl.GetUniqueId = (decltype(g_rccl.GetUniqueId))sym("ncclGetUniqueId");
  g_rccl.CommInitRank = (decltype(g_rccl.CommInitRank))sym("ncclCommInitRank");
  g_rccl.CommInitAll = (decltype(g_rccl.CommInitAll))sym("ncclCommInitAll");
  g_rccl.CommDestroy = (decltype(g_rccl.CommDestroy))sym("ncclCommDestroy");
  g_rccl.Reduce = (decltype(g_rccl.Reduce))sym("ncclReduce");
  g_rccl.GroupStart = (decltype(g_rccl.GroupStart))sym("ncclGroupStart");
  g_rccl.GroupEnd = (decltype(g_rccl.GroupEnd))sym("ncclGroupEnd");
  g_rccl.GetErrorString = (decltype(g_rccl.GetErrorString))sym("ncclGetErrorString");
  if (!ok) { dlclose(so); return false; }
  g_rccl.so = so;
  return true;
}
}

struct ptc_ctx {
  int device = 0;
  std::string err;
  LaunchCfg cfg{};
  uint32_t toplet_budget = 73;
  size_t max_batch_paths = (size_t)7 << 27;
  int timing = 1;
  std::vector<HostMaterial> mats;
  std::vector<HostMesh> meshes;
  std::vector<HostInstance> insts;
  std::vector<HostTexture> texs;
  HostEnv env;
  float cam_pos[3]{}, cam_target[3]{}, cam_fov = 0, cam_aspect = 1;
  bool have_cam = false;
  ptc_lens_params lens{0.0f, 1.0f, 0, 0.0f};
  int tex_linear = 0;
  int bvh_default = PTC_BVH_SAH;
  int bvh_builder = PTC_BVH_SAH;
  int device_builder = PTC_BVH_LBVH;
  bool committed = false;
  std::shared_ptr<HostBuilt> built = std::make_shared<HostBuilt>();
  CommittedScene scene;
  std::vector<MeshPose> poses;
  DevCamera cam{};
  bool debug_verts_from_device = false;
  int refit_on_device = 1;
  int trace_rays_per_lane = 8;
  int trace_overlap = 1;
  BuildScratch bscratch;
  std::vector<Lane> lanes;
  int n_lanes = 1;
  uint64_t batches_issued = 0;
  bool in_frame = false;
  DevFrame fr{};
  int spp_total = 0, integrator = 0;
  uint32_t samples_done = 0;
  uint32_t sample_base = 0;
  uint32_t resolve_divisor = 0;
  uint32_t pending = 0;
  uint32_t per_batch = 1;
  DevBuf<uint32_t> owned;
  bool owned_key_valid = false;
  int owned_w = 0, owned_h = 0, owned_rank = 0, owned_count = 0;
  uint32_t owned_n = 0;
  DevBuf<float4> accum, radiance;
  DevBuf<uint32_t> ldr;
  DevBuf<uint2> half;
  int rad_w = 0, rad_h = 0;
  DevBuf<float4> g_albedo, g_normal, g_pos, dn_cv[2], denoised;
  DevBuf<int32_t> g_prim;
  DevBuf<float2> g_uv;
  DevBuf<unsigned long long> g_stats;
  bool guides_valid = false, denoised_valid = false;
  int output = PTC_OUTPUT_RADIANCE;
  hipEvent_t ev_dn[4] = {nullptr, nullptr, nullptr, nullptr};
  bool ev_dn_recorded[2] = {false, false};
  bool adaptive = false;
  ptc_adaptive_params ad_params{};
  DevBuf<uint32_t> ad_pix[2], ad_slot[2], ad_count, ad_block, ad_n;
  DevBuf<float2> ad_mom;
  DevBuf<uint8_t> ad_flags, ad_keep;
  int ad_cur = 0;
  uint32_t ad_passes = 0;
  double ad_seconds = 0.0;
  hipEvent_t ev_ad[2] = {nullptr, nullptr};
  bool cov_setting = false, cov_on = false;
  bool cov_resolved = false;
  bool sv_valid = false;
  DevBuf<float4> ad_cov4, sv_colour, sv_var;
  DevBuf<float2> ad_cov2;
  size_t frame_batch_paths = 0;
  DevBuf<float4> tp_dn[2], tp_mom[2], tp_nz[2], tp_pk[2], tp_motion, tp_accum;
  DevBuf<float4> tp_snap;
  bool tp_snap_current = false;
  bool tp_live = false;
  int tp_cur = 0, tp_w = 0, tp_h = 0, tp_demodulate = 0;
  DevCamera tp_cam{};
  bool tp_accum_valid = false;
  hipEvent_t ev_tp[2] = {nullptr, nullptr};
  bool ev_tp_recorded = false;
  ncclComm_t comm = nullptr;
  int comm_rank = 0, comm_size = 0;
  bool comm_owned = true;
  ptc_stats stats{};
  std::vector<Span> spans;
  std::vector<hipEvent_t> free_events;
  size_t events_created = 0;
};

struct ptc_group {
  std::vector<ptc_ctx*> ctx;
  std::vector<ncclComm_t> comms;
  std::string err;
};

namespace {

constexpr size_t kQueueBytesPerPath = 176;
constexpr size_t kMaxSpans = 1024;
int fail(ptc_ctx* c, int code, const std::string& msg) { if (c) c->err = msg; return code; }
void drop_history(ptc_ctx* c) { c->tp_live = false; c->tp_snap_current = false; }
void drop_guides(ptc_ctx* c) { c->guides_valid = false; c->denoised_valid = false; c->tp_accum_valid = false; c->output = PTC_OUTPUT_RADIANCE; }
const float4* served_image(const ptc_ctx* c) { return c->output == PTC_OUTPUT_DENOISED ? c->denoised.p : c->output == PTC_OUTPUT_ACCUMULATED ? c->tp_accum.p : c->radiance.p; }
const char* const kNoDevice = "this context has no device (PTC_DEVICE_NONE): the call needs a gfx950 GPU; there is no CPU path";

#define HIP_TRY(c, expr)                                                                                 \
  do {                                                                                                   \
    hipError_t e_ = (expr);                                                                              \
    if (e_ != hipSuccess)                                                                                \
// ... 121 lines not shown

int ensure_overflow_slabs(ptc_ctx* c) {
  const int need = (int)c->built->max_depth + 2;
  const uint32_t ovf = (uint32_t)(need - c->cfg.stack_lds > 0 ? need - c->cfg.stack_lds : 1);
  if (ovf <= c->scene.dsc.ovf_depth) return PTC_OK;
  const size_t total_waves = (size_t)c->cfg.n_cu * (size_t)c->cfg.trace_blocks_per_cu * (size_t)(pt_trace_block_threads() / 64);
  for (auto& ln : c->lanes) {
    std::vector<void*> fresh;
    uint2 *a = nullptr, *b = nullptr;
    int rc = dev_alloc(c, fresh, &a, total_waves * ovf * 64);
    if (!rc && c->trace_overlap) rc = dev_alloc(c, fresh, &b, total_waves * ovf * 64);
    if (rc) { free_all(fresh); return rc; }
    ln.free_overflow_slabs();
    ln.stack_ovf = a; ln.stack_ovf2 = b;
  }
  c->scene.dsc.ovf_depth = ovf;
  return PTC_OK;
}

int configure_launch(ptc_ctx* c) {
  const int need = (int)c->built->max_depth + 2;
  int l = 6, per_cu = 0;
  bool l_forced = false;
  if (const char* e = std::getenv("PTC_STACK_LDS")) { int v = std::atoi(e); if (v >= 1 && v <= 64) { l = v; l_forced = true; } }
  if (l > need) l = need;
  size_t lds = 0;
  for (;; --l) {
    c->cfg.stack_lds = l;
    lds = pt_trace_lds_bytes(c->cfg, c->scene.dsc);
    if (lds > 160u * 1024u) { if (l > 1 && !l_forced) continue; return fail(c, PTC_E_ARG, "configure_launch: staged tree top + stack exceed the 160 KiB of LDS"); }
    per_cu = trace_blocks_per_cu_cached(lds);
    if (per_cu >= 8 || l <= 2 || l_forced) break;
  }
  if (per_cu < 1) return fail(c, PTC_E_DEVICE, "configure_launch: the trace kernels do not fit a CU with this LDS size");
  if (const char* e = std::getenv("PTC_TRACE_BLOCKS_PER_CU")) { int v = std::atoi(e); if (v >= 1 && v <= per_cu) per_cu = v; }
  c->cfg.trace_blocks_per_cu = per_cu;
  { int rc = ensure_overflow_slabs(c); if (rc) return rc; }
  if (c->trace_overlap)
    for (auto& ln : c->lanes)
      if (!ln.stream2 && hipStreamCreateWithFlags(&ln.stream2, hipStreamNonBlocking) != hipSuccess) return fail(c, PTC_E_DEVICE, "configure_launch: hipStreamCreate failed");
  return PTC_OK;
}

DevScene lane_scene(ptc_ctx* c, int l) { DevScene d = c->scene.dsc; d.stack_ovf = c->lanes[(size_t)l].stack_ovf; return d; }
int publish_lane_scenes(ptc_ctx* c, hipStream_t st) {
  for (int l = 0; l < c->n_lanes; ++l) {
    const DevScene ds = lane_scene(c, l);
    HIP_TRY(c, hipMemcpyAsync(c->lanes[(size_t)l].d_scene, &ds, sizeof ds, hipMemcpyHostToDevice, st));
  }
  return PTC_OK;
}
DevQueues batch_queues(ptc_ctx* c, int l, uint32_t n) {
  DevQueues q = c->lanes[(size_t)l].q;
  ptc_seg_layout(n, (uint32_t)c->cfg.shade_waves, q.n_seg, q.seg_len);
  return q;
}
bool is_raster(int integrator) { return integrator == PTC_INTEGRATOR_RASTER_COMPAT || integrator == PTC_INTEGRATOR_RASTER_GBUFFER16; }

LaunchCfg batch_cfg(const ptc_ctx* c, uint32_t n_paths) {
  LaunchCfg cfg = c->cfg;
  const uint64_t per_block = (uint64_t)pt_trace_block_threads() * (uint64_t)c->trace_rays_per_lane;
  uint64_t per_cu = ((uint64_t)n_paths + per_block * (uint64_t)cfg.n_cu - 1u) / (per_block * (uint64_t)cfg.n_cu);
  if (per_cu < 1) per_cu = 1;
  if (per_cu < (uint64_t)cfg.trace_blocks_per_cu) cfg.trace_blocks_per_cu = (int)per_cu;
  return cfg;
}

DevAdaptive dev_adaptive(const ptc_ctx* c) {
  return DevAdaptive{c->ad_mom.p, c->ad_count.p, c->ad_flags.p, c->ad_keep.p, c->ad_block.p, c->ad_n.p, c->cov_on ? c->ad_cov4.p : nullptr, c->cov_on ? c->ad_cov2.p : nullptr};
}

uint32_t batch_samples(const ptc_ctx* c, size_t n_pixels, size_t batch_paths) {
  size_t per = !n_pixels ? 1 : batch_paths / n_pixels / (size_t)c->n_lanes;
  if (per < 1) per = 1;
  if (per > 0x7fffffffu) per = 0x7fffffffu;
  {
    const uint64_t max_slots = 0xfffffff0ull - 64ull * (uint64_t)c->cfg.shade_waves - 64ull;
    if (n_pixels && (uint64_t)n_pixels * per > max_slots) per = max_slots / n_pixels;
    if (per < 1) per = 1;
  }
  return (uint32_t)per;
}

int run_batch(ptc_ctx* c, int l, uint32_t first_sample, uint32_t n_samples) {
  const uint32_t n_paths = c->fr.n_owned * n_samples;
  Lane& ln = c->lanes[(size_t)l];
  hipStream_t st = ln.stream;
  const DevQueues q = batch_queues(c, l, n_paths);
  const DevScene sc = lane_scene(c, l);
  const LaunchCfg cfg = batch_cfg(c, n_paths);
  if (c->spans.size() > kMaxSpans) {
    collect_times(c, false);
    if (c->spans.size() > kMaxSpans) { (void)hipEventSynchronize(c->spans[c->spans.size() - kMaxSpans].b); collect_times(c, false); }
  }
  ScopedSpan whole(c, st, 3);
  pt_launch_set_counts(st, cfg, q, n_paths, 0);
  if (is_raster(c->integrator)) {
    pt_launch_raygen(st, c->cam, c->fr, q, 0, 1, true);
    { ScopedSpan t(c, st, 0); pt_launch_trace_closest(st, cfg, sc, q, 0, true); c->stats.launches_trace_closest++; }
    pt_launch_shade_raster(st, sc, c->cam, c->fr, q, c->accum.p, c->integrator == PTC_INTEGRATOR_RASTER_GBUFFER16);
  } else {
    if (c->lens.aperture_radius > 0.0f) pt_launch_raygen_lens(st, c->cam, c->lens, c->fr, q, first_sample, n_samples);
    else pt_launch_raygen(st, c->cam, c->fr, q, first_sample, n_samples, false);
    const bool shadows = sc.n_lights > 0 || sc.env_ok;
    const bool small_batch = n_paths <= (1u << 26);
    const bool overlap = (c->trace_overlap == 2 || (c->trace_overlap == 1 && small_batch)) && shadows && ln.stream2 && ln.stack_ovf2;
    if (overlap) {
      const size_t need = (size_t)c->fr.max_bounces + 1;
      while (ln.ev_scan.size() < need) { hipEvent_t e = nullptr; HIP_TRY(c, hipEventCreateWithFlags(&e, hipEventDisableTiming)); ln.ev_scan.push_back(e); }
      while (ln.ev_any.size() < need) { hipEvent_t e = nullptr; HIP_TRY(c, hipEventCreateWithFlags(&e, hipEventDisableTiming)); ln.ev_any.push_back(e); }
    }
    DevScene sc_any = sc;
    if (overlap) sc_any.stack_ovf = ln.stack_ovf2;
    const bool per_kernel = !overlap || c->timing >= 2;
    for (int b = 0; b <= c->fr.max_bounces; ++b) {
      { ScopedSpan t(c, st, 0, per_kernel); pt_launch_trace_closest(st, cfg, sc, q, b & 1, false); c->stats.launches_trace_closest++; }
      if (overlap && b > 0) HIP_TRY(c, hipStreamWaitEvent(st, ln.ev_any[(size_t)b - 1], 0));
      { ScopedSpan t(c, st, 2, per_kernel); pt_launch_shade(st, cfg, ln.d_scene, c->fr, q, b & 1, (uint32_t)b); }
      if (b == c->fr.max_bounces) break;
      pt_launch_scan(st, cfg, q, (b + 1) & 1);
      if (overlap) {
        HIP_TRY(c, hipEventRecord(ln.ev_scan[(size_t)b], st));
        HIP_TRY(c, hipStreamWaitEvent(ln.stream2, ln.ev_scan[(size_t)b], 0));
        { ScopedSpan t(c, ln.stream2, 1, per_kernel); pt_launch_trace_any(ln.stream2, cfg, sc_any, q, nullptr); c->stats.launches_trace_any++; }
        HIP_TRY(c, hipEventRecord(ln.ev_any[(size_t)b], ln.stream2));
      } else if (shadows) {
        ScopedSpan t(c, st, 1); pt_launch_trace_any(st, cfg, sc, q, nullptr); c->stats.launches_trace_any++;
      }
    }
    if (c->n_lanes > 1 && c->batches_issued > 0) {
      const int prev = (int)((c->batches_issued - 1) % (uint64_t)c->n_lanes);
      if (prev != l) HIP_TRY(c, hipStreamWaitEvent(st, c->lanes[(size_t)prev].acc_done, 0));
    }
    if (c->adaptive) pt_launch_ad_accumulate(st, c->fr.n_owned, c->ad_slot[c->ad_cur].p, q.lpath, c->accum.p, dev_adaptive(c), n_samples);
    else pt_launch_accumulate(st, c->fr, q, c->accum.p, n_samples);
    if (c->n_lanes > 1) HIP_TRY(c, hipEventRecord(ln.acc_done, st));
  }
  c->batches_issued++;
  HIP_TRY(c, hipGetLastError());
  return PTC_OK;
}

int issue(ptc_ctx* c, uint32_t k) {
  if (is_raster(c->integrator)) {
    if (c->samples_done == 0) {
      int rc = ensure_lane_queues(c, c->fr.n_owned);
      if (rc) return rc;
      if ((rc = run_batch(c, 0, 0, 1))) return rc;
      c->stats.paths = c->fr.n_owned;
    }
    c->samples_done += k;
    return PTC_OK;
  }
  const uint64_t cap = (uint64_t)c->fr.n_owned * k;
  int rc = ensure_lane_queues(c, (uint32_t)cap);
  if (rc) return rc;
  if ((rc = run_batch(c, (int)(c->batches_issued % (uint64_t)c->n_lanes), c->sample_base + c->samples_done, k))) return rc;
  c->samples_done += k;
  c->stats.paths += cap;
  return PTC_OK;
}
int flush(ptc_ctx* c) {
  if (!c->in_frame) return PTC_OK;
  while (c->pending) {
    const uint32_t k = c->pending < c->per_batch ? c->pending : c->per_batch;
    c->pending -= k;
    if (c->fr.n_owned == 0) { c->samples_done += k; continue; }
    int rc = issue(c, k);
    if (rc) return rc;
  }
  return PTC_OK;
}

int join_lanes_on_stream0(ptc_ctx* c) {
  if (c->n_lanes > 1 && !is_raster(c->integrator))
    for (int l = 1; l < c->n_lanes; ++l)
      if ((uint64_t)l < c->batches_issued) HIP_TRY(c, hipStreamWaitEvent(c->lanes[0].stream, c->lanes[(size_t)l].acc_done, 0));
  return PTC_OK;
}

int temporal_keep_positions(ptc_ctx* c) {
  if (!c->tp_live || c->tp_snap_current || c->device < 0) return PTC_OK;
  const uint32_t n_prims = c->built->n_tris;
  int rc = ensure_buf(c, c->tp_snap, (size_t)3 * n_prims);
  if (rc) return rc;
  pt_launch_temporal_snapshot(c->lanes[0].stream, c->scene.dsc.shade, c->scene.dsc.shade_stride, n_prims, c->tp_snap.p);
  HIP_TRY(c, hipGetLastError());
  c->tp_snap_current = true;
  return PTC_OK;
}

int need_device(ptc_ctx* c) {
  if (!c) return PTC_E_ARG;
  if (c->device < 0) return fail(c, PTC_E_DEVICE, kNoDevice);
  HIP_TRY(c, hipSetDevice(c->device));
  return PTC_OK;
}

int sum_lane_stats(ptc_ctx* c, unsigned long long st[ST_N]) {
  for (int i = 0; i < ST_N; ++i) st[i] = 0;
  for (auto& ln : c->lanes) {
    if (!ln.q.stats) continue;
    unsigned long long one[ST_N * ST_STRIDE];
    HIP_TRY(c, hipMemcpy(one, ln.q.stats, sizeof one, hipMemcpyDeviceToHost));
    for (int i = 0; i < ST_N; ++i) st[i] += one[i * ST_STRIDE];
  }
  return PTC_OK;
}

int convert_half(ptc_ctx* c) {
  if (!c->radiance.p || c->rad_w == 0) return fail(c, PTC_E_STATE, "radiance_rgba16f: nothing rendered");
  const size_t n = (size_t)c->rad_w * c->rad_h;
  int rc = ensure_buf(c, c->half, n);
  if (rc) return rc;
  pt_launch_to_half(c->lanes[0].stream, served_image(c), c->half.p, (uint32_t)n);
  HIP_TRY(c, hipGetLastError());
  return PTC_OK;
}

int debug_prepare(ptc_ctx* c, uint32_t n, const char* who) {
  { int rd = need_device(c); if (rd) return rd; }
  if (!c->committed) return fail(c, PTC_E_STATE, std::string(who) + ": scene not committed");
  { int rf = flush(c); if (rf) return rf; }
  { int rs = sync_all_lanes(c); if (rs) return rs; }
  c->in_frame = false; c->pending = 0; drop_guides(c);
  int rc = ensure_lane_queues(c, n);
  if (rc) return rc;
  for (auto& ln : c->lanes) HIP_TRY(c, hipMemset(ln.q.stats, 0, ST_N * ST_STRIDE * sizeof(unsigned long long)));
  return PTC_OK;
}

}

extern "C" {

int ptc_abi_version(void) { return PTC_ABI_VERSION; }

#ifndef PTC_KERNEL_SHA
#define PTC_KERNEL_SHA "unknown"
#endif
const char* ptc_launch_policy(const ptc_ctx* c) {
  static thread_local std::string out;
  static const ptc_ctx defaults;
  const ptc_ctx& x = c ? *c : defaults;
  char buf[512];
  std::snprintf(buf, sizeof buf, " | stack_lds_max=6 segments_per_cu_default=64 nodelets=%u lanes=%d batch_paths=%zu trace_overlap=%d(<=2^26 paths) rays_per_lane=%d shade_sort=%d refit=%s bvh=%s",
                x.toplet_budget, x.n_lanes, x.max_batch_paths, x.trace_overlap, x.trace_rays_per_lane, x.cfg.shade_sort, x.refit_on_device ? "device" : "host",
                x.bvh_builder == PTC_BVH_LBVH ? "lbvh" : "sah");
  out = std::string(pt_kernel_policy()) + buf;
  if (c && c->committed && c->device >= 0) {
    std::snprintf(buf, sizeof buf, " | trace_blocks_per_cu=%d stack_lds=%d lds_units=%u ovf_depth=%u shade_segments=%d shade_tables_lds=%d", c->cfg.trace_blocks_per_cu, c->cfg.stack_lds,
                  c->scene.dsc.n_lds_units, c->scene.dsc.ovf_depth, c->cfg.shade_waves, c->cfg.shade_tables_lds);
    out += buf;
  }
  return out.c_str();
}

const char* ptc_build_info(void) { return "ptc abi " PTC_STR(PTC_ABI_VERSION) " gfx950 kernels-sha256 " PTC_KERNEL_SHA; }

ptc_ctx* ptc_create(int device_id) {
  if (device_id == PTC_DEVICE_NONE) {
    ptc_ctx* c = new ptc_ctx();
    c->device = PTC_DEVICE_NONE;
    if (const char* s = std::getenv("PTC_NODELETS")) c->toplet_budget = (uint32_t)std::strtoul(s, nullptr, 10);
    if (const char* s = std::getenv("PTC_BVH")) { if (std::strcmp(s, "lbvh") == 0) c->bvh_default = c->bvh_builder = PTC_BVH_LBVH; }
    if (const char* s = std::getenv("PTC_DEVICE_BVH")) { if (std::strcmp(s, "sah") == 0) c->device_builder = PTC_BVH_SAH; }
    return c;
  }
  int n = 0;
  hipError_t e = hipGetDeviceCount(&n);
  if (e != hipSuccess || n <= 0) { g_create_error = std::string("ptc_create: no HIP device (") + hipGetErrorString(e) + "); this library has no CPU path"; return nullptr; }
  if (device_id < 0 || device_id >= n) { g_create_error = "ptc_create: device id out of range"; return nullptr; }
  if ((e = hipSetDevice(device_id)) != hipSuccess) { g_create_error = std::string("ptc_create: hipSetDevice: ") + hipGetErrorString(e); return nullptr; }
  hipDeviceProp_t prop;
  if ((e = hipGetDeviceProperties(&prop, device_id)) != hipSuccess) { g_create_error = std::string("ptc_create: ") + hipGetErrorString(e); return nullptr; }
  if (std::string(prop.gcnArchName).rfind("gfx950", 0) != 0) { g_create_error = std::string("ptc_create: device is ") + prop.gcnArchName + ", this library is built for gfx950 only"; return nullptr; }
  ptc_ctx* c = new ptc_ctx();
  c->device = device_id;
  c->cfg.n_cu = prop.multiProcessorCount;
  c->cfg.trace_blocks_per_cu = 4;
  c->cfg.stack_lds = 6;
  {
    int per_cu = 64;
    if (const char* s = std::getenv("PTC_SEGMENTS_PER_CU")) { int v = std::atoi(s); if (v >= 1 && v <= 64) per_cu = v; }
    uint32_t n = (uint32_t)(c->cfg.n_cu * per_cu);
    c->cfg.shade_waves = (int)(n > PTC_MAX_SEGMENTS ? PTC_MAX_SEGMENTS : n);
  }
  if (const char* s = std::getenv("PTC_SHADE_SORT")) c->cfg.shade_sort = std::atoi(s) != 0 ? 1 : 0;
  if (const char* s = std::getenv("PTC_TRACE_RAYS_PER_LANE")) { int v = std::atoi(s); if (v >= 1 && v <= 4096) c->trace_rays_per_lane = v; }
  if (const char* s = std::getenv("PTC_TRACE_OVERLAP")) { int v = std::atoi(s); if (v >= 0 && v <= 2) c->trace_overlap = v; }
  if (const char* s = std::getenv("PTC_NODELETS")) c->toplet_budget = (uint32_t)std::strtoul(s, nullptr, 10);
  if (const char* s = std::getenv("PTC_BATCH_PATHS")) { size_t v = std::strtoull(s, nullptr, 10); if (v >= 1024) c->max_batch_paths = v; }
  if (const char* s = std::getenv("PTC_TIMING")) { const int v = std::atoi(s); c->timing = v < 0 ? 0 : (v > 2 ? 2 : v); }
  if (const char* s = std::getenv("PTC_BVH")) { if (std::strcmp(s, "lbvh") == 0) c->bvh_default = c->bvh_builder = PTC_BVH_LBVH; }
  if (const char* s = std::getenv("PTC_DEVICE_BVH")) { if (std::strcmp(s, "sah") == 0) c->device_builder = PTC_BVH_SAH; }
  if (const char* s = std::getenv("PTC_LANES")) { int v = std::atoi(s); if (v >= 1 && v <= 8) c->n_lanes = v; }
  c->lanes.resize((size_t)c->n_lanes);
  bool ok = true;
  for (auto& ln : c->lanes) {
    ok = ok && hipStreamCreateWithFlags(&ln.stream, hipStreamNonBlocking) == hipSuccess && hipEventCreateWithFlags(&ln.acc_done, hipEventDisableTiming) == hipSuccess;
    ok = ok && hipMalloc((void**)&ln.q.cnt, CNT_N * sizeof(uint32_t)) == hipSuccess && hipMalloc((void**)&ln.q.stats, ST_N * ST_STRIDE * sizeof(unsigned long long)) == hipSuccess;
    ok = ok && hipMemset(ln.q.cnt, 0, CNT_N * sizeof(uint32_t)) == hipSuccess && hipMemset(ln.q.stats, 0, ST_N * ST_STRIDE * sizeof(unsigned long long)) == hipSuccess;
    uint32_t* segs = nullptr;
    const size_t per = PTC_MAX_SEGMENTS + 64;
    ok = ok && hipMalloc((void**)&segs, 5 * per * sizeof(uint32_t)) == hipSuccess && hipMemset(segs, 0, 5 * per * sizeof(uint32_t)) == hipSuccess;
    if (ok) { ln.q.seg_ray[0] = segs; ln.q.seg_ray[1] = segs + per; ln.q.seg_sh = segs + 2 * per; ln.q.pre_ray = segs + 3 * per; ln.q.pre_sh = segs + 4 * per; }
    ok = ok && hipMalloc((void**)&ln.d_scene, sizeof(DevScene)) == hipSuccess;
  }
  if (!ok) { g_create_error = "ptc_create: could not create the lane streams / events / counters"; ptc_destroy(c); return nullptr; }
  return c;
}

void ptc_destroy(ptc_ctx* c) {
  if (!c) return;
  if (c->device < 0) { delete c; return; }
  (void)hipSetDevice(c->device);
  for (auto& ln : c->lanes) if (ln.stream) (void)hipStreamSynchronize(ln.stream);
  if (c->comm && c->comm_owned && g_rccl.so) (void)g_rccl.CommDestroy(c->comm);
  for (const Span& s : c->spans) { (void)hipEventDestroy(s.a); (void)hipEventDestroy(s.b); }
  for (hipEvent_t e : c->free_events) (void)hipEventDestroy(e);
  for (auto& ln : c->lanes) {
    if (ln.acc_done) (void)hipEventDestroy(ln.acc_done);
    free_all(ln.allocs);
    if (ln.q.cnt) (void)hipFree(ln.q.cnt);
    if (ln.q.stats) (void)hipFree(ln.q.stats);
    if (ln.q.seg_ray[0]) (void)hipFree(ln.q.seg_ray[0]);
    if (ln.d_scene) (void)hipFree(ln.d_scene);
    if (ln.stream) (void)hipStreamDestroy(ln.stream);
    if (ln.stream2) (void)hipStreamDestroy(ln.stream2);
    for (hipEvent_t e : ln.ev_scan) (void)hipEventDestroy(e);
    for (hipEvent_t e : ln.ev_any) (void)hipEventDestroy(e);
  }
  release_scene(c);
  if (c->bscratch.p) (void)hipFree(c->bscratch.p);
  c->owned.release(); c->accum.release(); c->radiance.release(); c->ldr.release(); c->half.release();
  c->g_albedo.release(); c->g_normal.release(); c->g_pos.release(); c->dn_cv[0].release(); c->dn_cv[1].release(); c->denoised.release();
  c->g_prim.release(); c->g_uv.release(); c->g_stats.release();
  for (hipEvent_t e : c->ev_dn) if (e) (void)hipEventDestroy(e);
  for (auto* b : {&c->ad_pix[0], &c->ad_pix[1], &c->ad_slot[0], &c->ad_slot[1], &c->ad_count, &c->ad_block, &c->ad_n}) b->release();
  c->ad_mom.release(); c->ad_flags.release(); c->ad_keep.release();
  c->ad_cov4.release(); c->ad_cov2.release(); c->sv_colour.release(); c->sv_var.release();
  for (hipEvent_t e : c->ev_ad) if (e) (void)hipEventDestroy(e);
  for (int k = 0; k < 2; ++k) { c->tp_dn[k].release(); c->tp_mom[k].release(); c->tp_nz[k].release(); c->tp_pk[k].release(); }
  c->tp_motion.release(); c->tp_accum.release(); c->tp_snap.release();
  for (hipEvent_t e : c->ev_tp) if (e) (void)hipEventDestroy(e);
  delete c;
}

const char* ptc_last_error(const ptc_ctx* c) { return c ? c->err.c_str() : g_create_error.c_str(); }

int ptc_scene_begin(ptc_ctx* c) {
  if (!c) return PTC_E_ARG;
  if (c->device >= 0) {
    HIP_TRY(c, hipSetDevice(c->device));
    { int rs = sync_all_lanes(c); if (rs) return rs; }
  }
  c->mats.clear(); c->meshes.clear(); c->insts.clear(); c->texs.clear(); c->env = HostEnv{}; c->tex_linear = 0;
  c->bvh_builder = c->bvh_default;
  c->poses.clear();
  c->have_cam = false; c->committed = false; c->in_frame = false; c->pending = 0; drop_guides(c);
  ptc_lens_default_params(&c->lens);
  drop_history(c);
  release_scene(c);
  return PTC_OK;
}

int ptc_add_material(ptc_ctx* c, const float base_color[4], float metallic, float roughness, const float emissive[3],
                     int tex_color, int tex_normal, int tex_mr) {
  if (!c) return PTC_E_ARG;
  if (!base_color || !emissive) return fail(c, PTC_E_ARG, "add_material: null pointer");
  const int nt = (int)c->texs.size();
// ... 975 lines not shown
  if (!out) return fail(c, PTC_E_ARG, "read_radiance: null pointer");
  if (!c->radiance.p || c->rad_w == 0) return fail(c, PTC_E_STATE, "read_radiance: nothing rendered");
  { int rs = sync_all_lanes(c); if (rs) return rs; }
  HIP_TRY(c, hipMemcpy(out, served_image(c), (size_t)c->rad_w * c->rad_h * sizeof(float4), hipMemcpyDeviceToHost));
  return PTC_OK;
}

void* ptc_radiance_device_ptr(ptc_ctx* c) { return (c && c->device >= 0) ? (void*)c->radiance.p : nullptr; }

int ptc_read_radiance_rgba16f(ptc_ctx* c, uint16_t* out) {
  { int rd = need_device(c); if (rd) return rd; }
  if (!out) return fail(c, PTC_E_ARG, "read_radiance_rgba16f: null pointer");
  { int rc = convert_half(c); if (rc) return rc; }
  HIP_TRY(c, hipStreamSynchronize(c->lanes[0].stream));
  HIP_TRY(c, hipMemcpy(out, c->half.p, (size_t)c->rad_w * c->rad_h * sizeof(uint2), hipMemcpyDeviceToHost));
  return PTC_OK;
}
void* ptc_radiance_rgba16f_device_ptr(ptc_ctx* c) {
  if (need_device(c)) return nullptr;
  if (convert_half(c)) return nullptr;
  if (hipStreamSynchronize(c->lanes[0].stream) != hipSuccess) return nullptr;
  return (void*)c->half.p;
}

int ptc_write_radiance_rgba32f(ptc_ctx* c, const float* in) {
  { int rd = need_device(c); if (rd) return rd; }
  if (!in) return fail(c, PTC_E_ARG, "write_radiance: null pointer");
  if (!c->radiance.p || c->rad_w == 0) return fail(c, PTC_E_STATE, "write_radiance: no frame");
  { int rs = sync_all_lanes(c); if (rs) return rs; }
  HIP_TRY(c, hipMemcpy(c->radiance.p, in, (size_t)c->rad_w * c->rad_h * sizeof(float4), hipMemcpyHostToDevice));
  return PTC_OK;
}

int ptc_tonemap_rgba8(ptc_ctx* c, uint8_t* out) {
  { int rd = need_device(c); if (rd) return rd; }
  if (!out) return fail(c, PTC_E_ARG, "tonemap: null pointer");
  if (!c->radiance.p || c->rad_w == 0) return fail(c, PTC_E_STATE, "tonemap: nothing rendered");
  int rc;
  if ((rc = ensure_buf(c, c->ldr, (size_t)c->rad_w * c->rad_h))) return rc;
  hipStream_t s0 = c->lanes[0].stream;
  pt_launch_tonemap(s0, served_image(c), c->ldr.p, c->rad_w, c->rad_h);
  HIP_TRY(c, hipGetLastError());
  HIP_TRY(c, hipStreamSynchronize(s0));
  HIP_TRY(c, hipMemcpy(out, c->ldr.p, (size_t)c->rad_w * c->rad_h * 4, hipMemcpyDeviceToHost));
  return PTC_OK;
}

namespace {
int ensure_dn_events(ptc_ctx* c) {
  for (hipEvent_t& e : c->ev_dn) if (!e) HIP_TRY(c, hipEventCreate(&e));
  return PTC_OK;
}
}

int ptc_frame_guides(ptc_ctx* c) {
  { int rd = need_device(c); if (rd) return rd; }
  if (!c->in_frame) return fail(c, PTC_E_STATE, "frame_guides: no frame");
  if (c->integrator != PTC_INTEGRATOR_PATH) return fail(c, PTC_E_STATE, "frame_guides: the frame is not a PTC_INTEGRATOR_PATH frame (the raster integrators are noise-free)");
  const uint32_t n = (uint32_t)c->fr.w * (uint32_t)c->fr.h;
  int rc;
  if ((rc = ensure_buf(c, c->g_albedo, n)) || (rc = ensure_buf(c, c->g_normal, n)) || (rc = ensure_buf(c, c->g_pos, n)) || (rc = ensure_buf(c, c->g_prim, n)) ||
      (rc = ensure_buf(c, c->g_uv, n)) || (rc = ensure_dn_events(c))) return rc;
  if (!c->g_stats.p) {
    if ((rc = ensure_buf(c, c->g_stats, (size_t)ST_N * ST_STRIDE))) return rc;
    HIP_TRY(c, hipMemset(c->g_stats.p, 0, ST_N * ST_STRIDE * sizeof(unsigned long long)));
  }
  {
    const uint32_t want = n < (1u << 21) ? n : (1u << 21);
    if (c->lanes[0].q.cap < want && (rc = ensure_lane_queues(c, want))) return rc;
  }
  Lane& ln = c->lanes[0];
  hipStream_t st = ln.stream;
  const DevScene sc = lane_scene(c, 0);
  const GuideBufs g = {c->g_albedo.p, c->g_normal.p, c->g_pos.p, c->g_prim.p, c->g_uv.p};
  const uint32_t chunk = ln.q.cap < n ? ln.q.cap : n;
  HIP_TRY(c, hipEventRecord(c->ev_dn[0], st));
  for (uint32_t first = 0; first < n; first += chunk) {
    const uint32_t m = n - first < chunk ? n - first : chunk;
    DevQueues q = batch_queues(c, 0, m);
    q.stats = c->g_stats.p;
    const LaunchCfg cfg = batch_cfg(c, m);
    pt_launch_set_counts(st, cfg, q, m, 0);
    pt_launch_raygen_guides(st, c->cam, c->fr.w, c->fr.h, first, m, q);
    pt_launch_trace_closest(st, cfg, sc, q, 0, false);
    pt_launch_guides(st, sc, c->cam, c->fr.w, c->fr.h, first, m, q, g);
  }
  HIP_TRY(c, hipEventRecord(c->ev_dn[1], st));
  HIP_TRY(c, hipGetLastError());
  c->ev_dn_recorded[0] = true;
  c->guides_valid = true;
  return PTC_OK;
}

int ptc_read_guide_rgba32f(ptc_ctx* c, int which, float* out) {
  { int rd = need_device(c); if (rd) return rd; }
  if (!out) return fail(c, PTC_E_ARG, "read_guide: null pointer");
  if (which != PTC_GUIDE_ALBEDO && which != PTC_GUIDE_NORMAL_DEPTH) return fail(c, PTC_E_ARG, "read_guide: unknown guide");
  if (!c->guides_valid) return fail(c, PTC_E_STATE, "read_guide: no guides (ptc_frame_guides)");
  HIP_TRY(c, hipStreamSynchronize(c->lanes[0].stream));
  HIP_TRY(c, hipMemcpy(out, which == PTC_GUIDE_ALBEDO ? c->g_albedo.p : c->g_normal.p, (size_t)c->rad_w * c->rad_h * sizeof(float4), hipMemcpyDeviceToHost));
  return PTC_OK;
}

int ptc_read_guide_hit(ptc_ctx* c, int32_t* prim, float* uv) {
  { int rd = need_device(c); if (rd) return rd; }
  if (!c->guides_valid) return fail(c, PTC_E_STATE, "read_guide_hit: no guides (ptc_frame_guides)");
  HIP_TRY(c, hipStreamSynchronize(c->lanes[0].stream));
  const size_t n = (size_t)c->rad_w * c->rad_h;
  if (prim) HIP_TRY(c, hipMemcpy(prim, c->g_prim.p, n * sizeof(int32_t), hipMemcpyDeviceToHost));
  if (uv) HIP_TRY(c, hipMemcpy(uv, c->g_uv.p, n * sizeof(float2), hipMemcpyDeviceToHost));
  return PTC_OK;
}

void ptc_denoise_default_params(ptc_denoise_params* p) {
  if (!p) return;
  p->iterations = 4; p->sigma_l = 4.0f; p->sigma_n = 128.0f; p->sigma_p = 1.0f; p->demodulate = 1;
}

namespace {
int denoise_image(ptc_ctx* c, const ptc_denoise_params* params, bool accumulated, bool sampled = false);
}
int ptc_denoise(ptc_ctx* c, const ptc_denoise_params* params) { return denoise_image(c, params, false); }
int ptc_denoise_accumulated(ptc_ctx* c, const ptc_denoise_params* params) { return denoise_image(c, params, true); }
int ptc_denoise_sampled(ptc_ctx* c, const ptc_denoise_params* params) { return denoise_image(c, params, false, true); }

namespace {
int denoise_image(ptc_ctx* c, const ptc_denoise_params* params, bool accumulated, bool sampled) {
  { int rd = need_device(c); if (rd) return rd; }
  ptc_denoise_params p;
  ptc_denoise_default_params(&p);
  if (params) p = *params;
  auto bad = [](float v) { return !(v >= 0.0f) || !(v <= 3.0e38f); };
  if (p.iterations < 0 || p.iterations > PTC_DENOISE_MAX_ITERATIONS) return fail(c, PTC_E_ARG, "denoise: iterations outside 0..8");
  if (bad(p.sigma_l) || bad(p.sigma_n) || bad(p.sigma_p)) return fail(c, PTC_E_ARG, "denoise: a sigma is negative or not finite");
  if (!c->guides_valid) return fail(c, PTC_E_STATE, "denoise: no valid guides (ptc_frame_guides after the frame's ptc_frame_begin)");
  if (!c->radiance.p || c->rad_w == 0) return fail(c, PTC_E_STATE, "denoise: no radiance buffer");
  if (accumulated && !c->tp_accum_valid) return fail(c, PTC_E_STATE, "denoise_accumulated: the frame has no accumulated image (ptc_temporal_accumulate)");
  if (accumulated && (p.demodulate ? 1 : 0) != c->tp_demodulate) return fail(c, PTC_E_ARG, "denoise_accumulated: demodulate differs from the accumulate's");
  if (sampled && !(c->in_frame && c->adaptive && c->cov_on)) return fail(c, PTC_E_STATE, "denoise_sampled: the frame is not an adaptive frame that keeps the sample covariance (ptc_set_sample_covariance before ptc_frame_set_adaptive)");
  if (sampled && (!c->cov_resolved || c->pending)) return fail(c, PTC_E_STATE, "denoise_sampled: samples were added since the last ptc_frame_resolve");
  const size_t n = (size_t)c->rad_w * c->rad_h;
  int rc;
  if ((rc = ensure_buf(c, c->denoised, n)) || (rc = ensure_dn_events(c))) return rc;
  if (sampled && ((rc = ensure_buf(c, c->sv_colour, n)) || (rc = ensure_buf(c, c->sv_var, n)))) return rc;
  if (p.iterations > 0 && ((rc = ensure_buf(c, c->dn_cv[0], n)) || (rc = ensure_buf(c, c->dn_cv[1], n)))) return rc;
  hipStream_t s0 = c->lanes[0].stream;
  HIP_TRY(c, hipEventRecord(c->ev_dn[2], s0));
  if (sampled)
    pt_launch_ad_sampled_variance(s0, c->owned_n, c->owned.p, c->accum.p, dev_adaptive(c), c->g_albedo.p, c->radiance.p, p.demodulate ? 1 : 0, c->sv_colour.p, c->sv_var.p,
                                  (uint32_t)n, (size_t)c->owned_n != n);
  if (p.iterations == 0) HIP_TRY(c, hipMemcpyAsync(c->denoised.p, accumulated ? c->tp_accum.p : c->radiance.p, n * sizeof(float4), hipMemcpyDeviceToDevice, s0));
  else {
    DenoiseArgs a{};
    a.w = c->rad_w; a.h = c->rad_h; a.sigma_l = p.sigma_l; a.sigma_n = p.sigma_n; a.sigma_p = p.sigma_p; a.demodulate = p.demodulate ? 1 : 0;
    a.pix = (2.0f * c->cam.sy) / (float)c->rad_h;
    a.radiance = c->radiance.p;
    a.g = GuideBufs{c->g_albedo.p, c->g_normal.p, c->g_pos.p, c->g_prim.p, c->g_uv.p};
    if (sampled) {
      DenoiseArgs ap = a;
      ap.demodulate = 0;
      pt_launch_denoise_prepare(s0, ap, c->sv_colour.p, c->sv_var.p, c->dn_cv[0].p);
    } else if (accumulated) {
      DenoiseArgs ap = a;
      ap.demodulate = 0;
      pt_launch_denoise_prepare(s0, ap, c->tp_dn[c->tp_cur].p, c->tp_mom[c->tp_cur].p, c->dn_cv[0].p);
    } else pt_launch_denoise_prepare(s0, a, c->radiance.p, nullptr, c->dn_cv[0].p);
    for (int i = 0; i < p.iterations; ++i) {
// ... 419 lines not shown
  const auto t0 = std::chrono::steady_clock::now();
  if (c0->device >= 0 && refit_on_device(c0)) {
    bool host_way = false;
    auto mine = std::make_shared<HostBuilt>(*c0->built);
    for (size_t i = 0; i < g->ctx.size() && !host_way; ++i) {
      ptc_ctx* c = g->ctx[i];
      if (hipSetDevice(c->device) != hipSuccess) { g->err = "ptc_group_scene_refit: hipSetDevice failed"; return PTC_E_DEVICE; }
      if (i) { c->insts = c0->insts; deform_take(c, c0, false); }
      c->built = mine;
      const int rc = device_refit(c, t0);
      if (rc > 0) { host_way = true; break; }
      if (rc) {
        g->err = "device " + std::to_string(i) + ": " + ptc_last_error(c);
        if (i == 0) return rc;
        host_way = true; break;
      }
    }
    if (!host_way) return PTC_OK;
  }
  auto built = std::make_shared<HostBuilt>(*c0->built);
  const size_t n_recs = built->recs.size(), n_shade = built->shade.size(), n_lights = built->lights.size(), n_cdf = built->cdf.size();
  deform_host_all(c0);
  const std::string e = ptc_refit_scene(c0->mats, c0->meshes, c0->insts, c0->texs, c0->env, *built);
  if (!e.empty()) { g->err = e; return PTC_E_STATE; }
  const bool same = built->recs.size() == n_recs && built->shade.size() == n_shade && built->lights.size() == n_lights && built->cdf.size() == n_cdf;
  for (size_t i = 0; i < g->ctx.size(); ++i) {
    ptc_ctx* c = g->ctx[i];
    if (c->device >= 0 && hipSetDevice(c->device) != hipSuccess) { g->err = "ptc_group_scene_refit: hipSetDevice failed"; return PTC_E_DEVICE; }
    if (i) { c->insts = c0->insts; deform_take(c, c0, true); }
    c->built = built;
    c->in_frame = false; c->pending = 0; drop_guides(c);
    int rc = c->device >= 0 ? refit_upload(c, same, t0) : PTC_OK;
    if (!rc) rc = deform_after_host_refit(c);
    if (rc) { g->err = "device " + std::to_string(i) + ": " + ptc_last_error(c); return rc; }
    c->stats.seconds_refit = std::chrono::duration<double>(std::chrono::steady_clock::now() - t0).count();
  }
  return PTC_OK;
}

int ptc_group_render(ptc_group* g, int w, int h, int spp, uint64_t seed, int max_bounces, int integrator) {
  if (!g || g->ctx.empty()) return PTC_E_ARG;
  const int n = (int)g->ctx.size();
  auto bail = [&](int i, int rc) { g->err = std::string("device ") + std::to_string(i) + ": " + ptc_last_error(g->ctx[(size_t)i]); return rc; };
  for (int i = 0; i < n; ++i) { int rc = ptc_frame_begin(g->ctx[(size_t)i], w, h, spp, seed, max_bounces, integrator, i, n); if (rc) return bail(i, rc); }
  for (int i = 0; i < n; ++i) { int rc = ptc_frame_add_samples(g->ctx[(size_t)i], spp); if (rc) return bail(i, rc); }
  for (int i = 0; i < n; ++i) { int rc = ptc_frame_resolve(g->ctx[(size_t)i]); if (rc) return bail(i, rc); }
  if (n > 1) {
    ncclResult_t r = g_rccl.GroupStart();
    for (int i = 0; i < n && r == ncclSuccess; ++i) {
      ptc_ctx* c = g->ctx[(size_t)i];
      if (hipSetDevice(c->device) != hipSuccess) { g->err = "ptc_group_render: hipSetDevice failed"; (void)g_rccl.GroupEnd(); return PTC_E_DEVICE; }
      r = g_rccl.Reduce(c->radiance.p, c->radiance.p, (size_t)w * h * 4, ncclFloat32, ncclSum, 0, c->comm, c->lanes[0].stream);
    }
    const ncclResult_t r2 = g_rccl.GroupEnd();
    if (r != ncclSuccess || r2 != ncclSuccess) { g->err = std::string("ptc_group_render: ncclReduce: ") + g_rccl.GetErrorString(r != ncclSuccess ? r : r2); return PTC_E_DEVICE; }
  }
  for (int i = 0; i < n; ++i) { int rc = ptc_sync(g->ctx[(size_t)i]); if (rc) return bail(i, rc); }
  return PTC_OK;
}

void ptc_group_destroy(ptc_group* g) {
  if (!g) return;
  for (ptc_ctx* c : g->ctx)
    if (c && c->device >= 0) { (void)hipSetDevice(c->device); for (auto& ln : c->lanes) if (ln.stream) (void)hipStreamSynchronize(ln.stream); }
  for (ncclComm_t cm : g->comms) if (cm && g_rccl.so) (void)g_rccl.CommDestroy(cm);
  for (ptc_ctx* c : g->ctx) { if (c) { c->comm = nullptr; ptc_destroy(c); } }
  delete g;
}

int ptc_debug_trace_closest(ptc_ctx* c, const float* origins, const float* dirs, uint32_t n, float* out_t, int32_t* out_prim, float* out_uv) {
  if (!c) return PTC_E_ARG;
  if (c->device >= 0 && (!origins || !dirs || !out_t || !out_prim || !out_uv || n == 0)) return fail(c, PTC_E_ARG, "debug_trace_closest: bad argument");
  { int rc = debug_prepare(c, n, "debug_trace_closest"); if (rc) return rc; }
  const Lane& ln = c->lanes[0];
  std::vector<float4> A(n), B(n);
  for (uint32_t i = 0; i < n; ++i) {
    A[i] = make_float4(origins[i * 3], origins[i * 3 + 1], origins[i * 3 + 2], dirs[i * 3]);
    B[i] = make_float4(dirs[i * 3 + 1], dirs[i * 3 + 2], 0.0f, 0.0f);
  }
  HIP_TRY(c, hipMemcpy(ln.q.ray[0].A, A.data(), n * sizeof(float4), hipMemcpyHostToDevice));
  HIP_TRY(c, hipMemcpy(ln.q.ray[0].B, B.data(), n * sizeof(float4), hipMemcpyHostToDevice));
  const DevQueues q = batch_queues(c, 0, n);
  pt_launch_set_counts(ln.stream, c->cfg, q, n, 0);
  pt_launch_trace_closest(ln.stream, c->cfg, lane_scene(c, 0), q, 0, false);
  HIP_TRY(c, hipGetLastError());
  HIP_TRY(c, hipStreamSynchronize(ln.stream));
  std::vector<float4> H(n);
  HIP_TRY(c, hipMemcpy(H.data(), ln.q.hit, n * sizeof(float4), hipMemcpyDeviceToHost));
  for (uint32_t i = 0; i < n; ++i) {
    int32_t pc; std::memcpy(&pc, &H[i].y, 4);
    out_t[i] = H[i].x; out_prim[i] = pc < 0 ? -1 : (pc & 0x0fffffff); out_uv[i * 2] = H[i].z; out_uv[i * 2 + 1] = H[i].w;
  }
  return PTC_OK;
}

int ptc_debug_trace_any(ptc_ctx* c, const float* origins, const float* dirs, const float* tmax, uint32_t n, uint8_t* out_occluded) {
  if (!c) return PTC_E_ARG;
  if (c->device >= 0 && (!origins || !dirs || !tmax || !out_occluded || n == 0)) return fail(c, PTC_E_ARG, "debug_trace_any: bad argument");
  { int rc = debug_prepare(c, n, "debug_trace_any"); if (rc) return rc; }
  const Lane& ln = c->lanes[0];
  std::vector<float4> A(n), B(n);
  for (uint32_t i = 0; i < n; ++i) {
    A[i] = make_float4(origins[i * 3], origins[i * 3 + 1], origins[i * 3 + 2], dirs[i * 3]);
    B[i] = make_float4(dirs[i * 3 + 1], dirs[i * 3 + 2], tmax[i], 0.0f);
  }
  HIP_TRY(c, hipMemcpy(ln.q.shadow.A, A.data(), n * sizeof(float4), hipMemcpyHostToDevice));
  HIP_TRY(c, hipMemcpy(ln.q.shadow.B, B.data(), n * sizeof(float4), hipMemcpyHostToDevice));
  uint8_t* d_out = nullptr;
  HIP_TRY(c, hipMalloc((void**)&d_out, n));
  const DevQueues q = batch_queues(c, 0, n);
  pt_launch_set_counts(ln.stream, c->cfg, q, 0, n);
  pt_launch_trace_any(ln.stream, c->cfg, lane_scene(c, 0), q, d_out);
  hipError_t e = hipGetLastError();
  if (e == hipSuccess) e = hipStreamSynchronize(ln.stream);
  if (e == hipSuccess) e = hipMemcpy(out_occluded, d_out, n, hipMemcpyDeviceToHost);
  (void)hipFree(d_out);
  if (e != hipSuccess) return fail(c, PTC_E_DEVICE, std::string("debug_trace_any: ") + hipGetErrorString(e));
  return PTC_OK;
}

int ptc_debug_lens_sample(const ptc_lens_params* lens, float u1, float u2, float out_xy[2]) {
  if (!lens || !out_xy || lens_params_error(*lens) || !(u1 >= 0.0f && u1 < 1.0f) || !(u2 >= 0.0f && u2 < 1.0f)) return PTC_E_ARG;
  pt_lens_point(*lens, u1, u2, out_xy[0], out_xy[1]);
  return PTC_OK;
}

int ptc_debug_camera_rays(ptc_ctx* c, int w, int h, uint64_t seed, uint32_t first_sample, uint32_t n_samples, const uint32_t* pixels, uint32_t n_pixels,
                          float* origins, float* dirs) {
  if (!c) return PTC_E_ARG;
  if (!pixels || !origins || !dirs || w <= 0 || h <= 0 || (uint64_t)w * (uint64_t)h > 0x7fffffffull || n_samples == 0 || n_pixels == 0 ||
      (uint64_t)n_pixels * (uint64_t)n_samples > 0x7fffffffull || (uint64_t)first_sample + n_samples > 0xffffffffull)
    return fail(c, PTC_E_ARG, "debug_camera_rays: bad argument");
  for (uint32_t j = 0; j < n_pixels; ++j)
    if (pixels[j] >= (uint32_t)w * (uint32_t)h) return fail(c, PTC_E_ARG, "debug_camera_rays: pixel index outside the frame");
  const uint32_t n = n_pixels * n_samples;
  const uint32_t seed_hash = frame_seed_hash(seed);
  if (c->device < 0) {
    if (!c->have_cam) return fail(c, PTC_E_STATE, "debug_camera_rays: no camera (ptc_set_camera)");
    DevCamera cam;
    ptc_make_camera(c->cam_pos, c->cam_target, c->cam_fov, c->cam_aspect, cam);
    for (uint32_t p = 0; p < n; ++p) {
      uint32_t key;
      pt_lens_ray(cam, c->lens, w, h, seed_hash, pixels[p % n_pixels], first_sample + p / n_pixels, origins + (size_t)p * 3, dirs + (size_t)p * 3, key);
    }
    return PTC_OK;
  }
  { int rc = debug_prepare(c, n, "debug_camera_rays"); if (rc) return rc; }
  const Lane& ln = c->lanes[0];
  DevBuf<uint32_t> list;
  { int rc = ensure_buf(c, list, n_pixels); if (rc) return rc; }
  std::vector<float4> A(n), B(n);
  hipError_t e = hipMemcpy(list.p, pixels, (size_t)n_pixels * 4, hipMemcpyHostToDevice);
  if (e == hipSuccess) {
    DevFrame fr{};
    fr.w = w; fr.h = h; fr.seed_hash = seed_hash; fr.max_bounces = 0; fr.n_owned = n_pixels; fr.owned = list.p;
    const DevQueues q = batch_queues(c, 0, n);
    if (c->lens.aperture_radius > 0.0f) pt_launch_raygen_lens(ln.stream, c->cam, c->lens, fr, q, first_sample, n_samples);
    else pt_launch_raygen(ln.stream, c->cam, fr, q, first_sample, n_samples, false);
    e = hipGetLastError();
  }
  if (e == hipSuccess) e = hipStreamSynchronize(ln.stream);
  if (e == hipSuccess) e = hipMemcpy(A.data(), ln.q.ray[0].A, (size_t)n * sizeof(float4), hipMemcpyDeviceToHost);
  if (e == hipSuccess) e = hipMemcpy(B.data(), ln.q.ray[0].B, (size_t)n * sizeof(float4), hipMemcpyDeviceToHost);
  list.release();
  if (e != hipSuccess) return fail(c, PTC_E_DEVICE, std::string("debug_camera_rays: ") + hipGetErrorString(e));
  for (size_t p = 0; p < n; ++p) {
    origins[p * 3] = A[p].x; origins[p * 3 + 1] = A[p].y; origins[p * 3 + 2] = A[p].z;
    dirs[p * 3] = A[p].w; dirs[p * 3 + 1] = B[p].x; dirs[p * 3 + 2] = B[p].y;
  }
  return PTC_OK;
}

int ptc_debug_get_flat_scene(ptc_ctx* c, uint32_t* n_verts, uint32_t* n_tris, ptc_vertex* verts, uint32_t* indices, int32_t* tri_material) {
  if (!c) return PTC_E_ARG;
  if (!c->committed) return fail(c, PTC_E_STATE, "debug_get_flat_scene: scene not committed");
  { int rr = refresh_host_copy(c); if (rr) return rr; }
  const HostBuilt& B = *c->built;
  if (n_verts) *n_verts = (uint32_t)B.wverts.size();
  if (n_tris) *n_tris = B.n_tris;
  if (verts) std::memcpy(verts, B.wverts.data(), B.wverts.size() * sizeof(ptc_vertex));
  if (indices) std::memcpy(indices, B.widx.data(), B.widx.size() * 4);
  if (tri_material) std::memcpy(tri_material, B.tri_mat.data(), B.tri_mat.size() * 4);
  return PTC_OK;
}

int ptc_debug_get_description(ptc_ctx* c, int* n_materials, int* n_textures) {
  if (!c) return PTC_E_ARG;
  if (n_materials) *n_materials = (int)c->mats.size();
  if (n_textures) *n_textures = (int)c->texs.size();
  return PTC_OK;
}

int ptc_debug_get_material(ptc_ctx* c, int index, float out_factors[9], int out_textures[3]) {
  if (!c) return PTC_E_ARG;
  if (index < 0 || (size_t)index >= c->mats.size() || !out_factors || !out_textures) return fail(c, PTC_E_ARG, "debug_get_material: bad argument");
  const HostMaterial& m = c->mats[(size_t)index];
  std::memcpy(out_factors, m.base, 16); out_factors[4] = m.metallic; out_factors[5] = m.roughness; std::memcpy(out_factors + 6, m.emissive, 12);
  out_textures[0] = m.tex_color; out_textures[1] = m.tex_normal; out_textures[2] = m.tex_mr;
  return PTC_OK;
}

int ptc_debug_get_texture(ptc_ctx* c, int index, int* w, int* h, uint8_t* rgba) {
  if (!c) return PTC_E_ARG;
  if (index < 0 || (size_t)index >= c->texs.size()) return fail(c, PTC_E_ARG, "debug_get_texture: bad argument");
  const HostTexture& t = c->texs[(size_t)index];
  if (w) *w = t.w;
  if (h) *h = t.h;
  if (rgba) std::memcpy(rgba, t.px.data(), t.px.size());
  return PTC_OK;
}

int ptc_debug_get_counters(ptc_ctx* c, uint64_t* out, int n) {
  { int rd = need_device(c); if (rd) return rd; }
  if (!out || n <= 0) return fail(c, PTC_E_ARG, "debug_get_counters: bad argument");
  { int rf = flush(c); if (rf) return rf; }
  { int rs = sync_all_lanes(c); if (rs) return rs; }
  unsigned long long st[ST_N];
  { int rc = sum_lane_stats(c, st); if (rc) return rc; }
  for (int i = 0; i < n; ++i) out[i] = i < ST_N ? st[i] : 0;
  return ST_N;
}

int ptc_debug_get_bvh(ptc_ctx* c, uint32_t* n_nodes, uint32_t* n_tris, uint32_t* n_units, float* units, float grid[6]) {
  if (!c) return PTC_E_ARG;
  if (!c->committed) return fail(c, PTC_E_STATE, "debug_get_bvh: scene not committed");
  { int rr = refresh_host_copy(c); if (rr) return rr; }
  const HostBuilt& B = *c->built;
  if (n_nodes) *n_nodes = B.n_nodes;
  if (n_tris) *n_tris = B.n_tri_records;
  if (n_units) *n_units = B.n_units;
  if (units) std::memcpy(units, B.recs.data(), B.recs.size() * 4);
  if (grid) for (int k = 0; k < 3; ++k) { grid[k] = B.grid_lo[k]; grid[3 + k] = B.grid_step[k]; }
  return PTC_OK;
}

uint64_t ptc_debug_host_build_id(const ptc_ctx* c) { return c ? (uint64_t)(uintptr_t)c->built.get() : 0u; }

int ptc_debug_get_internals(ptc_ctx* c, uint64_t out[8]) {
  if (!c || !out) return PTC_E_ARG;
  for (int i = 0; i < 8; ++i) out[i] = 0;
  out[0] = c->events_created; out[1] = c->spans.size(); out[2] = c->lanes.empty() ? 0 : c->lanes[0].q.cap; out[3] = c->per_batch; out[4] = c->pending;
// ... 76 lines not shown
```

physically-based-renderer_amd/csrc/ptc_internal.h:

```cpp
#pragma once
#include <hip/hip_runtime.h>
#include <stdint.h>

#include <memory>
#include <string>
#include <vector>

struct DevScene {
  const float4* recs;
  float grid_lo[3], grid_step[3];
  const float4* shade;
  uint32_t shade_stride;
  const float4* mats;
  const uint32_t* texels;
  const int4* tex_info;
  const uint4* set_texels;
  const int4* set_info;
  int tex_linear;
  const float4* env;
  const float* env_marg;
  const float* env_cond;
  const uint16_t* env_marg_guide;
  const uint16_t* env_cond_guide;
  int env_w, env_h, env_ok;
  const float4* lights;
  const float* cdf;
  uint32_t n_lights;
  uint32_t n_mats;
  uint32_t n_lds_units;
  uint2* stack_ovf;
  uint32_t ovf_depth;
  float ray_eps;
};

struct DevCamera { float pos[3], f[3], s[3], u[3], sx, sy; };

struct DevFrame {
  int w, h;
  uint32_t seed_hash;
  int max_bounces;
  uint32_t n_owned;
  const uint32_t* owned;
};

struct RayQ { float4* A; float4* B; float4* C; };
struct ShadowQ { float4* A; float4* B; float4* C; };

struct DevQueues {
  RayQ ray[2];
  ShadowQ shadow;
  float4* hit;
  float4* lpath;
  uint32_t* cnt;
  uint32_t* seg_ray[2];
  uint32_t* seg_sh;
  uint32_t* pre_ray;
  uint32_t* pre_sh;
  unsigned long long* stats;
  uint32_t cap;
  uint32_t n_seg, seg_len;
};

enum { CNT_RAY_TOTAL = 0, CNT_RAY_CHUNK, CNT_RAY_NCHUNKS, CNT_SH_TOTAL, CNT_SH_CHUNK, CNT_SH_NCHUNKS, CNT_WORK_TRACE = 32, CNT_WORK_SHADOW = 64, CNT_N = 96 };
#define PTC_MAX_SEGMENTS 16384u
#define PTC_ENV_GUIDE 256u
#define PTC_MATERIAL_CLASSES 8
#define ST_STRIDE 16
enum { ST_SEGMENTS = 0, ST_SHADOW, ST_HITS, ST_NODES_C, ST_TRIS_C, ST_NODES_A, ST_TRIS_A,
       ST_DIAG_NODE_ITERS, ST_DIAG_TRI_ITERS, ST_DIAG_LEAF_VISITS, ST_DIAG_ROUNDS, ST_DIAG_REFILLED, ST_N };

#define PTC_SEG_MIN_LEN 512u
inline void ptc_seg_layout(uint32_t n, uint32_t max_seg, uint32_t& n_seg, uint32_t& seg_len) {
  uint32_t s = (n + PTC_SEG_MIN_LEN - 1u) / PTC_SEG_MIN_LEN;
  if (s > max_seg) s = max_seg;
  if (s < 1u) s = 1u;
  const uint32_t per = (n + s - 1u) / s;
  n_seg = s; seg_len = per ? ((per + 63u) & ~63u) : 64u;
}
inline size_t ptc_seg_slots(uint32_t cap, uint32_t max_seg) { return (size_t)cap + 64u * (size_t)max_seg + 64u; }

struct LaunchCfg { int n_cu; int trace_blocks_per_cu; int stack_lds;  int shade_waves;
                   int shade_sort;
                   int shade_tables_lds;  };

const char* pt_kernel_policy();
int pt_trace_block_threads();
size_t pt_trace_lds_bytes(const LaunchCfg&, const DevScene&);
int pt_trace_blocks_per_cu(size_t lds_bytes);
void pt_launch_set_counts(hipStream_t, const LaunchCfg&, const DevQueues&, uint32_t n_rays, uint32_t n_shadow);
void pt_launch_scan(hipStream_t, const LaunchCfg&, const DevQueues&, int qi_next);
int pt_shade_block_threads();
bool pt_shade_tables_fit(const DevScene&);
void pt_launch_raygen(hipStream_t, const DevCamera&, const DevFrame&, const DevQueues&, uint32_t first_sample, uint32_t n_samples, bool raster);
void pt_launch_trace_closest(hipStream_t, const LaunchCfg&, const DevScene&, const DevQueues&, int qi, bool cull);
void pt_launch_shade(hipStream_t, const LaunchCfg&, const DevScene* scene_on_device, const DevFrame&, const DevQueues&, int qi, uint32_t bounce);
void pt_launch_trace_any(hipStream_t, const LaunchCfg&, const DevScene&, const DevQueues&, uint8_t* debug_out );
void pt_launch_accumulate(hipStream_t, const DevFrame&, const DevQueues&, float4* accum, uint32_t n_samples);
void pt_launch_shade_raster(hipStream_t, const DevScene&, const DevCamera&, const DevFrame&, const DevQueues&, float4* accum, bool gbuffer16);
void pt_launch_to_half(hipStream_t, const float4* radiance, uint2* out_rgba16f, uint32_t n_pixels);
void pt_launch_resolve(hipStream_t, const DevFrame&, const float4* accum, float4* radiance, float inv_spp_divisor, bool raster);
void pt_launch_tonemap(hipStream_t, const float4* radiance, uint32_t* rgba8, int w, int h);
struct GuideBufs { float4* albedo_class; float4* normal_depth; float4* pos_class; int32_t* prim; float2* uv; };
void pt_launch_raygen_guides(hipStream_t, const DevCamera&, int w, int h, uint32_t first_pixel, uint32_t n, const DevQueues&);
void pt_launch_guides(hipStream_t, const DevScene&, const DevCamera&, int w, int h, uint32_t first_pixel, uint32_t n, const DevQueues&, const GuideBufs&);

struct HostMaterial { float base[4]; float metallic, roughness; float emissive[3]; int tex_color, tex_normal, tex_mr; };
struct HostVertex { float position[3], normal[3], tangent[4], texcoord[2]; };
struct HostTexture { std::vector<uint8_t> px; int w, h; };
struct HostEnv { std::vector<float> rgb; int w = 0, h = 0; };
struct HostMesh { std::vector<HostVertex> v; std::vector<uint32_t> idx; int material; };
struct HostInstance { int mesh; float m[16]; };

struct HostBuilt {
  uint32_t n_wverts = 0;
  std::vector<HostVertex> wverts;
  std::vector<uint32_t> widx;
  std::vector<int32_t> tri_mat;
  std::vector<int32_t> prim_light;
  std::vector<float> shade;
  uint32_t shade_stride = 5;
  std::vector<uint32_t> texels;
  std::vector<int32_t> tex_info;
  std::vector<uint32_t> set_texels;
  std::vector<int32_t> set_info;
  std::vector<uint16_t> env_marg_guide, env_cond_guide;
  std::vector<float> env, env_marg, env_cond;
  int env_w = 0, env_h = 0, env_ok = 0;
  std::vector<float> recs;
  float grid_lo[3] = {0, 0, 0}, grid_step[3] = {1, 1, 1};
  std::vector<float> mats;
  std::vector<float> lights;
  std::vector<float> cdf;
  uint32_t n_nodes = 0, n_tris = 0, n_tri_records = 0, n_lights = 0, max_depth = 0, n_units = 0, n_lds_units = 0;
  float ray_eps = 0.0f;
  uint64_t sa_cost_fixed = 0;
  float sa_unit = 0.0f;
  std::shared_ptr<void> topology;
};

std::string ptc_build_scene(const std::vector<HostMaterial>&, const std::vector<HostMesh>&, const std::vector<HostInstance>&,
                            const std::vector<HostTexture>&, const HostEnv&, uint32_t toplet_budget, int bvh_builder ,
                            HostBuilt& out);
std::string ptc_build_skeleton(const std::vector<HostMaterial>&, const std::vector<HostMesh>&, const std::vector<HostInstance>&,
                               const std::vector<HostTexture>&, const HostEnv&, uint32_t toplet_budget, HostBuilt& out);
std::string ptc_refit_scene(const std::vector<HostMaterial>&, const std::vector<HostMesh>&, const std::vector<HostInstance>&,
                            const std::vector<HostTexture>&, const HostEnv&, HostBuilt& out);
void ptc_prim_classes(const std::vector<HostMaterial>&, const std::vector<int32_t>& tri_mat, std::vector<uint32_t>& out);
void ptc_trs_to_matrix(const float t[3], const float q_wxyz[4], const float s[3], float m16[16]);
void ptc_make_camera(const float pos[3], const float target[3], float fov, float aspect, DevCamera& cam);
void ptc_owned_pixels(int w, int h, int tile_rank, int tile_count, std::vector<uint32_t>& out);
```

Baseline: 1339.

## Use a slim 16-byte camera ray record for primary bounce

Primary camera rays now store only direction plus RNG key in one float4, instead of three float4s plus an lpath init. The shared camera origin is passed to the trace kernel as a kernel argument. Shade at bounce 0 derives path index, throughput and pdf implicitly and writes lpath directly rather than doing a read-modify-write. This cuts raygen writes and trace and shade reads for the first bounce, and skips the origin shuffles during trace. It adds extra template instantiations, which could change register allocation, and it is disabled for the lens, sort and raster paths.

```diff
diff --git a/physically-based-renderer_amd/csrc/pt_kernels.hip b/physically-based-renderer_amd/csrc/pt_kernels.hip
--- a/physically-based-renderer_amd/csrc/pt_kernels.hip
+++ b/physically-based-renderer_amd/csrc/pt_kernels.hip
@@ -100,27 +100,34 @@
 }
 
 template <bool RASTER>
-__global__ __launch_bounds__(256) void k_raygen(DevCamera cam, DevFrame fr, DevQueues q, uint32_t first_sample, uint32_t n_paths) {
-  const uint32_t p = blockIdx.x * 256u + threadIdx.x;
-  if (p >= n_paths) return;
+PT_DEV v3 camera_ray(const DevCamera& cam, const DevFrame& fr, uint32_t first_sample, uint32_t p, uint32_t& key, float& dvx, float& dvy) {
   const uint32_t j = p % fr.n_owned, sl = p / fr.n_owned;
   const uint32_t pixel = fr.owned[j];
   const uint32_t px = pixel % (uint32_t)fr.w, py = pixel / (uint32_t)fr.w;
   const uint32_t sample = first_sample + sl;
-  const uint32_t key = path_key(fr.seed_hash, pixel, sample);
+  key = path_key(fr.seed_hash, pixel, sample);
   float jx = 0.5f, jy = 0.5f;
   if (!RASTER) { jx = rng_f(key, 0, 0); jy = rng_f(key, 0, 1); }
   const float fx = ((float)px + jx) / (float)fr.w, fy = ((float)py + jy) / (float)fr.h;
-  const float dvx = (2.0f * fx - 1.0f) * cam.sx, dvy = (2.0f * fy - 1.0f) * cam.sy;
+  dvx = (2.0f * fx - 1.0f) * cam.sx; dvy = (2.0f * fy - 1.0f) * cam.sy;
   const v3 cs = V3(cam.s[0], cam.s[1], cam.s[2]), cu = V3(cam.u[0], cam.u[1], cam.u[2]), cf = V3(cam.f[0], cam.f[1], cam.f[2]);
-  const v3 d = normalize3(vfma(cs, dvx, vfma(cu, dvy, cf)));
+  return normalize3(vfma(cs, dvx, vfma(cu, dvy, cf)));
+}
+template <bool RASTER, bool SLIM>
+__global__ __launch_bounds__(256) void k_raygen(DevCamera cam, DevFrame fr, DevQueues q, uint32_t first_sample, uint32_t n_paths) {
+  static_assert(!(RASTER && SLIM), "the raster integrators keep the full record (clip interval in B.zw)");
+  const uint32_t p = blockIdx.x * 256u + threadIdx.x;
+  if (p >= n_paths) return;
+  uint32_t key; float dvx, dvy;
+  const v3 d = camera_ray<RASTER>(cam, fr, first_sample, p, key, dvx, dvy);
+  const RayQ& r = q.ray[0];
+  if (SLIM) { r.A[p] = make_float4(d.x, d.y, d.z, __uint_as_float(key)); return; }
   float bz = 1.0f, bw = 1.0f;
   if (RASTER) {
     const float len = pt_sqrt(pt_fma(dvy, dvy, pt_fma(dvx, dvx, 1.0f)));
     const float dnear = (2.0f * PT_ZFAR * PT_ZNEAR) / (PT_ZFAR + PT_ZNEAR);
     bz = dnear * len; bw = PT_ZFAR * len;
   }
-  const RayQ& r = q.ray[0];
   r.A[p] = make_float4(cam.pos[0], cam.pos[1], cam.pos[2], d.x);
   r.B[p] = make_float4(d.y, d.z, bz, bw);
   r.C[p] = make_float4(1.0f, 0.0f, __uint_as_float(p), __uint_as_float(key));
@@ -320,13 +327,16 @@
   lds_u32* f;
   uint32_t n;
   PT_DEV void init(uint32_t* base) { f = (lds_u32*)base; n = 0; }
-  PT_DEV void stage(Reservoir& res, const DevQueues& q, const uint32_t* pre, const uint32_t* seg, uint32_t* ctr, const float4* QA, const float4* QB, uint32_t lane) {
+  template <bool CAM>
+  PT_DEV void stage(Reservoir& res, const DevQueues& q, const uint32_t* pre, const uint32_t* seg, uint32_t* ctr, const float4* QA, const float4* QB, v3 org, uint32_t lane) {
     uint32_t first;
     const uint32_t k = res.take(q, pre, seg, ctr, lane, TRACE_RING, first);
     if (lane < k) {
       const uint32_t ri = first + lane;
-      const float4 A = QA[ri], B = QB[ri];
-      const ray_t r = make_ray(V3(A.x, A.y, A.z), V3(A.w, B.x, B.y));
+      const float4 A = QA[ri];
+      ray_t r;
+      if (CAM) r = make_ray(org, V3(A.x, A.y, A.z));
+      else { const float4 B = QB[ri]; r = make_ray(V3(A.x, A.y, A.z), V3(A.w, B.x, B.y)); }
       f[lane] = ri;
       f[TRACE_RING + lane] = __float_as_uint(r.inv.x); f[2 * TRACE_RING + lane] = __float_as_uint(r.inv.y); f[3 * TRACE_RING + lane] = __float_as_uint(r.inv.z);
       f[4 * TRACE_RING + lane] = (r.inv.x >= 0.0f ? 1u : 0u) | (r.inv.y >= 0.0f ? 2u : 0u) | (r.inv.z >= 0.0f ? 4u : 0u);
@@ -376,8 +386,9 @@
   a = make_float4(x.x, x.y, x.z, x.w); b = make_float4(y.x, y.y, y.z, y.w); c = make_float4(z.x, z.y, z.z, z.w);
 }
 
-template <bool CULL>
-__global__ __launch_bounds__(TRACE_BLOCK, TRACE_MIN_WAVES) void k_trace_closest(DevScene sc, DevQueues q, int qi, int stack_lds) {
+template <bool CULL, bool CAM>
+__global__ __launch_bounds__(TRACE_BLOCK, TRACE_MIN_WAVES) void k_trace_closest(DevScene sc, DevQueues q, int qi, int stack_lds, float ox, float oy, float oz) {
+  static_assert(!(CULL && CAM), "culled rays carry their interval in B.zw: full record only");
   extern __shared__ float4 lds_raw[];
   __shared__ uint8_t s_pair[2][TRACE_WAVES][64];
   const uint32_t lane = lane_id();
@@ -407,6 +418,7 @@
   int cur = CUR_DONE;
   uint32_t ri = 0, oct = 0, gbase = 0, gmask = 0, tbase = 0, tmask = 0;
   ray_t r = make_ray(V3(0, 0, 0), V3(0, 0, 1));
+  if (CAM) r.o = V3(ox, oy, oz);
   float tmin = 0.0f, best_t = PT_T_INF, best_u = 0.0f, best_v = 0.0f;
   int best_prim = 0x7fffffff, best_cls = 0;
   bool found = false;
@@ -419,15 +431,18 @@
         while (mi) {
           if (ring.n == 0u) {
             if (res.exhausted) break;
-            ring.stage(res, q, q.pre_ray, seg_cnt, &q.cnt[CNT_WORK_TRACE], rq.A, rq.B, lane);
+            ring.stage<CAM>(res, q, q.pre_ray, seg_cnt, &q.cnt[CNT_WORK_TRACE], rq.A, rq.B, V3(ox, oy, oz), lane);
             if (ring.n == 0u) break;
           }
           v3 inv = V3(0, 0, 0); uint32_t oc = 0;
           const bool got = ring.pop(idle, ri, inv, oc);
           nr += (unsigned long long)__popcll(__ballot(got));
           if (got) {
-            const float4 A = rq.A[ri], Bq = rq.B[ri];
-            r.o = V3(A.x, A.y, A.z); r.d = V3(A.w, Bq.x, Bq.y); r.inv = inv;
+            const float4 A = rq.A[ri];
+            float4 Bq = make_float4(0, 0, 0, 0);
+            if (CAM) r.d = V3(A.x, A.y, A.z);
+            else { Bq = rq.B[ri]; r.o = V3(A.x, A.y, A.z); r.d = V3(A.w, Bq.x, Bq.y); }
+            r.inv = inv;
             oct = oc;
             tmin = CULL ? Bq.z : 0.0f;
             best_t = CULL ? Bq.w : PT_T_INF; best_u = 0.0f; best_v = 0.0f; best_prim = 0x7fffffff; best_cls = 0; found = false;
@@ -506,7 +521,8 @@
           const uint32_t task = dl.helper ? (uint32_t)tab_task[dl.rank_free] : lane;
           const int src = (int)(task & 63u);
           ray_t rr;
-          rr.o = V3(__shfl(r.o.x, src), __shfl(r.o.y, src), __shfl(r.o.z, src));
+          if (CAM) rr.o = r.o;
+          else rr.o = V3(__shfl(r.o.x, src), __shfl(r.o.y, src), __shfl(r.o.z, src));
           rr.d = V3(__shfl(r.d.x, src), __shfl(r.d.y, src), __shfl(r.d.z, src));
           uint32_t k = k1;
 #pragma unroll
@@ -581,7 +597,8 @@
           __builtin_amdgcn_fence(__ATOMIC_ACQUIRE, "wavefront");
           const int src = helper ? (int)tab_owner[rank_free] : (int)lane;
           ray_t rr;
-          rr.o = V3(__shfl(r.o.x, src), __shfl(r.o.y, src), __shfl(r.o.z, src));
+          if (CAM) rr.o = r.o;
+          else rr.o = V3(__shfl(r.o.x, src), __shfl(r.o.y, src), __shfl(r.o.z, src));
           rr.d = V3(__shfl(r.d.x, src), __shfl(r.d.y, src), __shfl(r.d.z, src));
           const uint32_t k2_src = (uint32_t)__shfl((int)k2, src);
           const uint32_t k = helper ? k2_src : k1;
@@ -682,7 +699,7 @@
         while (mi) {
           if (ring.n == 0u) {
             if (res.exhausted) break;
-            ring.stage(res, q, q.pre_sh, q.seg_sh, &q.cnt[CNT_WORK_SHADOW], q.shadow.A, q.shadow.B, lane);
+            ring.stage<false>(res, q, q.pre_sh, q.seg_sh, &q.cnt[CNT_WORK_SHADOW], q.shadow.A, q.shadow.B, V3(0, 0, 0), lane);
             if (ring.n == 0u) break;
           }
           v3 inv = V3(0, 0, 0); uint32_t oc = 0;
@@ -1032,8 +1049,10 @@
   __builtin_amdgcn_wave_barrier();
   __builtin_amdgcn_fence(__ATOMIC_ACQUIRE, "wavefront");
 }
-template <bool SORT, bool TABLES_LDS>
-__global__ __launch_bounds__(SHADE_BLOCK, SHADE_MIN_WAVES) void k_shade(const DevScene* __restrict__ scp, DevFrame fr, DevQueues q, int qi, uint32_t b) {
+template <bool SORT, bool TABLES_LDS, bool CAM>
+__global__ __launch_bounds__(SHADE_BLOCK, SHADE_MIN_WAVES) void k_shade(const DevScene* __restrict__ scp, DevFrame fr, DevQueues q, int qi, uint32_t bounce) {
+  static_assert(!(SORT && CAM), "the material sort keeps the full record");
+  const uint32_t b = CAM ? 0u : bounce;
   __shared__ float4 s_light[SHADE_LDS_LIGHTS * 5];
   __shared__ float s_cdf[SHADE_LDS_LIGHTS];
   __shared__ float4 s_mat[SHADE_LDS_MATS * 4];
@@ -1150,21 +1169,25 @@
     float4 oA, oB, oC, sA, sB, sC;
     oA = oB = oC = sA = sB = sC = make_float4(0, 0, 0, 0);
     if (valid) {
-      const float4 A = rin.A[slot], Bq = rin.B[slot], Cq = rin.C[slot], H = q.hit[slot];
-      const v3 d = V3(A.w, Bq.x, Bq.y);
-      v3 T = V3(Bq.z, Bq.w, Cq.x);
-      const float prev_pdf = Cq.y;
-      const uint32_t path = __float_as_uint(Cq.z), key = __float_as_uint(Cq.w);
+      const float4 A = rin.A[slot], H = q.hit[slot];
+      v3 d, T; float prev_pdf; uint32_t path, key;
+      if (CAM) { d = V3(A.x, A.y, A.z); T = V3(1.0f, 1.0f, 1.0f); prev_pdf = 0.0f; path = slot; key = __float_as_uint(A.w); }
+      else {
+        const float4 Bq = rin.B[slot], Cq = rin.C[slot];
+        d = V3(A.w, Bq.x, Bq.y); T = V3(Bq.z, Bq.w, Cq.x); prev_pdf = Cq.y; path = __float_as_uint(Cq.z); key = __float_as_uint(Cq.w);
+      }
       const float ht = H.x, hu = H.z, hv = H.w;
       if (__float_as_int(H.y) < 0) {
+        float4 L = make_float4(0.0f, 0.0f, 0.0f, 0.0f);
         if (SORT || has_env) {
         v3 Le; float pe; env_lookup(sc, d, Le, pe);
         float wgt = 1.0f;
         if (b > 0u) { const float pl = pe * p_env; const float pb2 = prev_pdf * prev_pdf; wgt = pb2 / pt_fma(pl, pl, pb2); }
-        float4 L = q.lpath[path];
+        if (!CAM) L = q.lpath[path];
         L.x = pt_fma(T.x * Le.x, wgt, L.x); L.y = pt_fma(T.y * Le.y, wgt, L.y); L.z = pt_fma(T.z * Le.z, wgt, L.z);
-        q.lpath[path] = L;
-        }
+        if (!CAM) q.lpath[path] = L;
+        }
+        if (CAM) q.lpath[path] = L;
       } else {
       const uint32_t prim = (uint32_t)__float_as_int(H.y) & ((1u << HIT_CLASS_SHIFT) - 1u);
       const size_t rec = (size_t)prim * sc.shade_stride;
@@ -1203,6 +1226,7 @@
       if (!front) { ng = -ng; ns = -ns; }
       if (!(dot3(ns, wo) > 0.0f)) ns = ng;
       const int li = __float_as_int(r1.w);
+      float4 L = make_float4(0.0f, 0.0f, 0.0f, 0.0f);
       if (li >= 0 && front) {
         const float4 l0 = ld4(lights, (size_t)(li * 5 + 0)), l1 = ld4(lights, (size_t)(li * 5 + 1)), l4 = ld4(lights, (size_t)(li * 5 + 4));
         float wgt = 1.0f;
@@ -1212,10 +1236,11 @@
           const float pb2 = prev_pdf * prev_pdf;
           wgt = pb2 / pt_fma(pl, pl, pb2);
         }
-        float4 L = q.lpath[path];
+        if (!CAM) L = q.lpath[path];
         L.x = pt_fma(T.x * l4.x, wgt, L.x); L.y = pt_fma(T.y * l4.y, wgt, L.y); L.z = pt_fma(T.z * l4.z, wgt, L.z);
-        q.lpath[path] = L;
-      }
+        if (!CAM) q.lpath[path] = L;
+      }
+      if (CAM) q.lpath[path] = L;
       if ((int)b < fr.max_bounces) {
         const bsdf_t bs = make_bsdf(V3(base_c[0], base_c[1], base_c[2]), metallic, roughness, lambert);
         v3 tx, ty; onb(ns, tx, ty);
@@ -1433,7 +1458,8 @@
 size_t pt_trace_lds_bytes(const LaunchCfg& cfg, const DevScene& sc) { return trace_lds_bytes(cfg, sc, true); }
 
 int pt_trace_blocks_per_cu(size_t lds) {
-  const void* fns[] = {(const void*)k_trace_closest<false>, (const void*)k_trace_closest<true>, (const void*)k_trace_any<false>, (const void*)k_trace_any<true>};
+  const void* fns[] = {(const void*)k_trace_closest<false, false>, (const void*)k_trace_closest<true, false>, (const void*)k_trace_closest<false, true>,
+                       (const void*)k_trace_any<false>, (const void*)k_trace_any<true>};
   int best = 1 << 30;
   for (const void* f : fns) {
     if (lds > 64u * 1024u && hipFuncSetAttribute(f, hipFuncAttributeMaxDynamicSharedMemorySize, (int)lds) != hipSuccess) return -1;
@@ -1453,18 +1479,20 @@
 }
 int pt_shade_block_threads() { return SHADE_BLOCK; }
 
-void pt_launch_raygen(hipStream_t s, const DevCamera& cam, const DevFrame& fr, const DevQueues& q, uint32_t first_sample, uint32_t n_samples, bool raster) {
+void pt_launch_raygen(hipStream_t s, const DevCamera& cam, const DevFrame& fr, const DevQueues& q, uint32_t first_sample, uint32_t n_samples, bool raster, bool slim) {
   const uint32_t n_paths = fr.n_owned * n_samples;
   const dim3 grid((n_paths + 255u) / 256u);
-  if (raster) hipLaunchKernelGGL(k_raygen<true>, grid, dim3(256), 0, s, cam, fr, q, first_sample, n_paths);
-  else hipLaunchKernelGGL(k_raygen<false>, grid, dim3(256), 0, s, cam, fr, q, first_sample, n_paths);
-}
-
-void pt_launch_trace_closest(hipStream_t s, const LaunchCfg& cfg, const DevScene& sc, const DevQueues& q, int qi, bool cull) {
+  if (raster) hipLaunchKernelGGL((k_raygen<true, false>), grid, dim3(256), 0, s, cam, fr, q, first_sample, n_paths);
+  else if (slim) hipLaunchKernelGGL((k_raygen<false, true>), grid, dim3(256), 0, s, cam, fr, q, first_sample, n_paths);
+  else hipLaunchKernelGGL((k_raygen<false, false>), grid, dim3(256), 0, s, cam, fr, q, first_sample, n_paths);
+}
+
+void pt_launch_trace_closest(hipStream_t s, const LaunchCfg& cfg, const DevScene& sc, const DevQueues& q, int qi, bool cull, const DevCamera* slim_cam) {
   const dim3 grid((unsigned)(cfg.n_cu * cfg.trace_blocks_per_cu));
   const size_t lds = trace_lds_bytes(cfg, sc, true);
-  if (cull) hipLaunchKernelGGL(k_trace_closest<true>, grid, dim3(TRACE_BLOCK), lds, s, sc, q, qi, cfg.stack_lds);
-  else hipLaunchKernelGGL(k_trace_closest<false>, grid, dim3(TRACE_BLOCK), lds, s, sc, q, qi, cfg.stack_lds);
+  if (slim_cam) hipLaunchKernelGGL((k_trace_closest<false, true>), grid, dim3(TRACE_BLOCK), lds, s, sc, q, qi, cfg.stack_lds, slim_cam->pos[0], slim_cam->pos[1], slim_cam->pos[2]);
+  else if (cull) hipLaunchKernelGGL((k_trace_closest<true, false>), grid, dim3(TRACE_BLOCK), lds, s, sc, q, qi, cfg.stack_lds, 0.0f, 0.0f, 0.0f);
+  else hipLaunchKernelGGL((k_trace_closest<false, false>), grid, dim3(TRACE_BLOCK), lds, s, sc, q, qi, cfg.stack_lds, 0.0f, 0.0f, 0.0f);
 }
 
 void pt_launch_trace_any(hipStream_t s, const LaunchCfg& cfg, const DevScene& sc, const DevQueues& q, uint8_t* debug_out) {
@@ -1474,11 +1502,16 @@
   else hipLaunchKernelGGL(k_trace_any<false>, grid, dim3(TRACE_BLOCK), lds, s, sc, q, cfg.stack_lds, debug_out);
 }
 
-void pt_launch_shade(hipStream_t s, const LaunchCfg& cfg, const DevScene* sc, const DevFrame& fr, const DevQueues& q, int qi, uint32_t bounce) {
+void pt_launch_shade(hipStream_t s, const LaunchCfg& cfg, const DevScene* sc, const DevFrame& fr, const DevQueues& q, int qi, uint32_t bounce, bool slim) {
   const dim3 grid((q.n_seg + SHADE_WAVES - 1u) / SHADE_WAVES);
-  if (cfg.shade_sort) hipLaunchKernelGGL((k_shade<true, false>), grid, dim3(SHADE_BLOCK), 0, s, sc, fr, q, qi, bounce);
-  else if (cfg.shade_tables_lds) hipLaunchKernelGGL((k_shade<false, true>), grid, dim3(SHADE_BLOCK), 0, s, sc, fr, q, qi, bounce);
-  else hipLaunchKernelGGL((k_shade<false, false>), grid, dim3(SHADE_BLOCK), 0, s, sc, fr, q, qi, bounce);
+  if (cfg.shade_sort) hipLaunchKernelGGL((k_shade<true, false, false>), grid, dim3(SHADE_BLOCK), 0, s, sc, fr, q, qi, bounce);
+  else if (cfg.shade_tables_lds) {
+    if (slim) hipLaunchKernelGGL((k_shade<false, true, true>), grid, dim3(SHADE_BLOCK), 0, s, sc, fr, q, qi, bounce);
+    else hipLaunchKernelGGL((k_shade<false, true, false>), grid, dim3(SHADE_BLOCK), 0, s, sc, fr, q, qi, bounce);
+  } else {
+    if (slim) hipLaunchKernelGGL((k_shade<false, false, true>), grid, dim3(SHADE_BLOCK), 0, s, sc, fr, q, qi, bounce);
+    else hipLaunchKernelGGL((k_shade<false, false, false>), grid, dim3(SHADE_BLOCK), 0, s, sc, fr, q, qi, bounce);
+  }
 }
 bool pt_shade_tables_fit(const DevScene& sc) {
   return sc.n_lights <= SHADE_LDS_LIGHTS && sc.n_mats <= SHADE_LDS_MATS && (!sc.env_ok || sc.env_h <= (int)SHADE_LDS_ENV_ROWS);
diff --git a/physically-based-renderer_amd/csrc/ptc_api.cpp b/physically-based-renderer_amd/csrc/ptc_api.cpp
--- a/physically-based-renderer_amd/csrc/ptc_api.cpp
+++ b/physically-based-renderer_amd/csrc/ptc_api.cpp
@@ -146,6 +146,7 @@
   DevCamera cam{};
   bool debug_verts_from_device = false;
   int refit_on_device = 1;
+  int camera_record_slim = 1;
   int trace_rays_per_lane = 8;
   int trace_overlap = 1;
   BuildScratch bscratch;
@@ -433,6 +434,8 @@
   return (uint32_t)per;
 }
 
+bool slim_camera_record(const ptc_ctx* c) { return c->camera_record_slim && !(c->lens.aperture_radius > 0.0f) && !c->cfg.shade_sort; }
+
 int run_batch(ptc_ctx* c, int l, uint32_t first_sample, uint32_t n_samples) {
   const uint32_t n_paths = c->fr.n_owned * n_samples;
   Lane& ln = c->lanes[(size_t)l];
@@ -447,12 +450,13 @@
   ScopedSpan whole(c, st, 3);
   pt_launch_set_counts(st, cfg, q, n_paths, 0);
   if (is_raster(c->integrator)) {
-    pt_launch_raygen(st, c->cam, c->fr, q, 0, 1, true);
-    { ScopedSpan t(c, st, 0); pt_launch_trace_closest(st, cfg, sc, q, 0, true); c->stats.launches_trace_closest++; }
+    pt_launch_raygen(st, c->cam, c->fr, q, 0, 1, true, false);
+    { ScopedSpan t(c, st, 0); pt_launch_trace_closest(st, cfg, sc, q, 0, true, nullptr); c->stats.launches_trace_closest++; }
     pt_launch_shade_raster(st, sc, c->cam, c->fr, q, c->accum.p, c->integrator == PTC_INTEGRATOR_RASTER_GBUFFER16);
   } else {
+    const bool slim = slim_camera_record(c);
     if (c->lens.aperture_radius > 0.0f) pt_launch_raygen_lens(st, c->cam, c->lens, c->fr, q, first_sample, n_samples);
-    else pt_launch_raygen(st, c->cam, c->fr, q, first_sample, n_samples, false);
+    else pt_launch_raygen(st, c->cam, c->fr, q, first_sample, n_samples, false, slim);
     const bool shadows = sc.n_lights > 0 || sc.env_ok;
     const bool small_batch = n_paths <= (1u << 26);
     const bool overlap = (c->trace_overlap == 2 || (c->trace_overlap == 1 && small_batch)) && shadows && ln.stream2 && ln.stack_ovf2;
@@ -465,9 +469,9 @@
     if (overlap) sc_any.stack_ovf = ln.stack_ovf2;
     const bool per_kernel = !overlap || c->timing >= 2;
     for (int b = 0; b <= c->fr.max_bounces; ++b) {
-      { ScopedSpan t(c, st, 0, per_kernel); pt_launch_trace_closest(st, cfg, sc, q, b & 1, false); c->stats.launches_trace_closest++; }
+      { ScopedSpan t(c, st, 0, per_kernel); pt_launch_trace_closest(st, cfg, sc, q, b & 1, false, slim && b == 0 ? &c->cam : nullptr); c->stats.launches_trace_closest++; }
       if (overlap && b > 0) HIP_TRY(c, hipStreamWaitEvent(st, ln.ev_any[(size_t)b - 1], 0));
-      { ScopedSpan t(c, st, 2, per_kernel); pt_launch_shade(st, cfg, ln.d_scene, c->fr, q, b & 1, (uint32_t)b); }
+      { ScopedSpan t(c, st, 2, per_kernel); pt_launch_shade(st, cfg, ln.d_scene, c->fr, q, b & 1, (uint32_t)b, slim && b == 0); }
       if (b == c->fr.max_bounces) break;
       pt_launch_scan(st, cfg, q, (b + 1) & 1);
       if (overlap) {
@@ -595,9 +599,9 @@
   static const ptc_ctx defaults;
   const ptc_ctx& x = c ? *c : defaults;
   char buf[512];
-  std::snprintf(buf, sizeof buf, " | stack_lds_max=6 segments_per_cu_default=64 nodelets=%u lanes=%d batch_paths=%zu trace_overlap=%d(<=2^26 paths) rays_per_lane=%d shade_sort=%d refit=%s bvh=%s",
+  std::snprintf(buf, sizeof buf, " | stack_lds_max=6 segments_per_cu_default=64 nodelets=%u lanes=%d batch_paths=%zu trace_overlap=%d(<=2^26 paths) rays_per_lane=%d shade_sort=%d refit=%s bvh=%s camera_record=%s",
                 x.toplet_budget, x.n_lanes, x.max_batch_paths, x.trace_overlap, x.trace_rays_per_lane, x.cfg.shade_sort, x.refit_on_device ? "device" : "host",
-                x.bvh_builder == PTC_BVH_LBVH ? "lbvh" : "sah");
+                x.bvh_builder == PTC_BVH_LBVH ? "lbvh" : "sah", slim_camera_record(&x) ? "slim" : "full");
   out = std::string(pt_kernel_policy()) + buf;
   if (c && c->committed && c->device >= 0) {
     std::snprintf(buf, sizeof buf, " | trace_blocks_per_cu=%d stack_lds=%d lds_units=%u ovf_depth=%u shade_segments=%d shade_tables_lds=%d", c->cfg.trace_blocks_per_cu, c->cfg.stack_lds,
@@ -638,6 +642,7 @@
     c->cfg.shade_waves = (int)(n > PTC_MAX_SEGMENTS ? PTC_MAX_SEGMENTS : n);
   }
   if (const char* s = std::getenv("PTC_SHADE_SORT")) c->cfg.shade_sort = std::atoi(s) != 0 ? 1 : 0;
+  if (const char* s = std::getenv("PTC_CAMERA_RECORD")) { if (std::strcmp(s, "full") == 0) c->camera_record_slim = 0; }
   if (const char* s = std::getenv("PTC_TRACE_RAYS_PER_LANE")) { int v = std::atoi(s); if (v >= 1 && v <= 4096) c->trace_rays_per_lane = v; }
   if (const char* s = std::getenv("PTC_TRACE_OVERLAP")) { int v = std::atoi(s); if (v >= 0 && v <= 2) c->trace_overlap = v; }
   if (const char* s = std::getenv("PTC_NODELETS")) c->toplet_budget = (uint32_t)std::strtoul(s, nullptr, 10);
@@ -1779,7 +1784,7 @@
     const LaunchCfg cfg = batch_cfg(c, m);
     pt_launch_set_counts(st, cfg, q, m, 0);
     pt_launch_raygen_guides(st, c->cam, c->fr.w, c->fr.h, first, m, q);
-    pt_launch_trace_closest(st, cfg, sc, q, 0, false);
+    pt_launch_trace_closest(st, cfg, sc, q, 0, false, nullptr);
     pt_launch_guides(st, sc, c->cam, c->fr.w, c->fr.h, first, m, q, g);
   }
   HIP_TRY(c, hipEventRecord(c->ev_dn[1], st));
@@ -2365,7 +2370,7 @@
   HIP_TRY(c, hipMemcpy(ln.q.ray[0].B, B.data(), n * sizeof(float4), hipMemcpyHostToDevice));
   const DevQueues q = batch_queues(c, 0, n);
   pt_launch_set_counts(ln.stream, c->cfg, q, n, 0);
-  pt_launch_trace_closest(ln.stream, c->cfg, lane_scene(c, 0), q, 0, false);
+  pt_launch_trace_closest(ln.stream, c->cfg, lane_scene(c, 0), q, 0, false, nullptr);
   HIP_TRY(c, hipGetLastError());
   HIP_TRY(c, hipStreamSynchronize(ln.stream));
   std::vector<float4> H(n);
@@ -2439,7 +2444,7 @@
     fr.w = w; fr.h = h; fr.seed_hash = seed_hash; fr.max_bounces = 0; fr.n_owned = n_pixels; fr.owned = list.p;
     const DevQueues q = batch_queues(c, 0, n);
     if (c->lens.aperture_radius > 0.0f) pt_launch_raygen_lens(ln.stream, c->cam, c->lens, fr, q, first_sample, n_samples);
-    else pt_launch_raygen(ln.stream, c->cam, fr, q, first_sample, n_samples, false);
+    else pt_launch_raygen(ln.stream, c->cam, fr, q, first_sample, n_samples, false, false);
     e = hipGetLastError();
   }
   if (e == hipSuccess) e = hipStreamSynchronize(ln.stream);
diff --git a/physically-based-renderer_amd/csrc/ptc_internal.h b/physically-based-renderer_amd/csrc/ptc_internal.h
--- a/physically-based-renderer_amd/csrc/ptc_internal.h
+++ b/physically-based-renderer_amd/csrc/ptc_internal.h
@@ -91,9 +91,9 @@
 void pt_launch_scan(hipStream_t, const LaunchCfg&, const DevQueues&, int qi_next);
 int pt_shade_block_threads();
 bool pt_shade_tables_fit(const DevScene&);
-void pt_launch_raygen(hipStream_t, const DevCamera&, const DevFrame&, const DevQueues&, uint32_t first_sample, uint32_t n_samples, bool raster);
-void pt_launch_trace_closest(hipStream_t, const LaunchCfg&, const DevScene&, const DevQueues&, int qi, bool cull);
-void pt_launch_shade(hipStream_t, const LaunchCfg&, const DevScene* scene_on_device, const DevFrame&, const DevQueues&, int qi, uint32_t bounce);
+void pt_launch_raygen(hipStream_t, const DevCamera&, const DevFrame&, const DevQueues&, uint32_t first_sample, uint32_t n_samples, bool raster, bool slim);
+void pt_launch_trace_closest(hipStream_t, const LaunchCfg&, const DevScene&, const DevQueues&, int qi, bool cull, const DevCamera* slim_cam );
+void pt_launch_shade(hipStream_t, const LaunchCfg&, const DevScene* scene_on_device, const DevFrame&, const DevQueues&, int qi, uint32_t bounce, bool slim);
 void pt_launch_trace_any(hipStream_t, const LaunchCfg&, const DevScene&, const DevQueues&, uint8_t* debug_out );
 void pt_launch_accumulate(hipStream_t, const DevFrame&, const DevQueues&, float4* accum, uint32_t n_samples);
 void pt_launch_shade_raster(hipStream_t, const DevScene&, const DevCamera&, const DevFrame&, const DevQueues&, float4* accum, bool gbuffer16);
```

New measurement: 1347, median of 6. About the same (+0.6%).
